# 10XGenomics/rust-pseudoaligner

Measured on AMD Instinct MI355X. Metric: reads/sec pseudoaligned (whole node) on synthetic 150bp reads, higher is better.
Workload: dtype u64; 1 GPU; config3: ~202k-transcript synthetic GENCODE-scale index (K=24), error-free 150bp reads; read_len=150, k=24, transcripts=201914, kmers=103866252, index_bytes=7185579820

## Files before the change

rust-pseudoaligner_amd/csrc/device_flatten.cpp:

```cpp
#include "device_flatten.hpp"

#include <algorithm>
#include <atomic>
#include <thread>

#include "dict_slots.hpp"
#include "lane_steps.hpp"
#include "pa_common.hpp"

#ifndef PA_BRANCH_TAILS
#define PA_BRANCH_TAILS 1
#endif

namespace pa {

DevIndexView FlatDevice::host_view() const {
    DevIndexView v;
    v.table = table.data();
    v.nbuckets = nbuckets;
    v.blobs = blobs.data();
    v.ledge = ledge.data();
    v.seg_g = seg_g.data();
    v.seg_nid = seg_nid.data();
    v.ec = ec.data();
    v.class_ref = class_ref.data();
    v.class_len = class_len.data();
    v.wtable = wtable.data();
    v.wbuckets = wbuckets;
    v.kmask = kmer_mask(k);
    v.kmask_hi = k > 32 ? kmer_mask(k - 32) : 0;
    v.k = k;
    v.num_nodes = num_nodes;
    v.num_classes = num_classes;
    v.num_segs = (uint32_t)seg_g.size();
    v.stream_nt = 0;
    v.bitmap_min = bitmap_min;
    v.bitmap_words = bitmap_words;
    return v;
}

namespace {

template <class F>
void par_ranges(int threads, uint64_t n, F f) {
    if (threads <= 1 || n < 4096) { f(0, n, 0); return; }
    std::vector<std::thread> th;
    for (int t = 0; t < threads; ++t) th.emplace_back([=] { f(n * t / threads, n * (t + 1) / threads, t); });
    for (auto& x : th) x.join();
}

template <class KT> struct Dict;

template <>
struct Dict<u128> {
    static constexpr double LOAD = 1.0 / 3.0;
    static constexpr uint32_t SLOTS = 2;
    uint32_t* words;
    uint64_t nbuckets;
    uint64_t bucket_of(u128 kmer) const { return ((pa_mix128((uint64_t)kmer, (uint64_t)(kmer >> 64)) >> 32) * (uint64_t)(uint32_t)nbuckets) >> 32; }
    void insert_mt(u128 kmer, uint32_t handle, uint32_t off) {
        uint64_t b = bucket_of(kmer);
        for (;;) {
            uint32_t* line = words + b * BUCKET_WORDS;
            for (uint32_t i = 0; i < SLOTS; ++i) {
                uint32_t expect = NO_HANDLE;
                if (__atomic_compare_exchange_n(&line[8 * i + 4], &expect, handle, false, __ATOMIC_RELAXED, __ATOMIC_RELAXED)) {
                    line[8 * i] = (uint32_t)kmer; line[8 * i + 1] = (uint32_t)(kmer >> 32);
                    line[8 * i + 2] = (uint32_t)(kmer >> 64); line[8 * i + 3] = (uint32_t)(kmer >> 96);
                    line[8 * i + 5] = off;
                    return;
                }
            }
            if (++b == nbuckets) b = 0;
        }
    }
    void insert_rest_mt(u128, uint32_t, uint32_t) {}
    bool find(u128 kmer, uint32_t& handle, uint32_t& off, uint32_t* probes_out = nullptr) const {
        uint64_t b = bucket_of(kmer);
        for (uint64_t probes = 0; probes < nbuckets; ++probes) {
            const uint32_t* line = words + b * BUCKET_WORDS;
            bool full = true;
            for (uint32_t i = 0; i < SLOTS; ++i) {
                if (line[8 * i + 4] == NO_HANDLE) { full = false; continue; }
                if (line[8 * i] == (uint32_t)kmer && line[8 * i + 1] == (uint32_t)(kmer >> 32) && line[8 * i + 2] == (uint32_t)(kmer >> 64) &&
                    line[8 * i + 3] == (uint32_t)(kmer >> 96)) {
                    handle = line[8 * i + 4];
                    off = line[8 * i + 5];
                    if (probes_out) *probes_out = (uint32_t)probes;
                    return true;
                }
            }
            if (!full) return false;
            if (++b == nbuckets) b = 0;
        }
        return false;
    }
};

struct HostAtomics {
    static bool cas(uint32_t* p, uint32_t expect, uint32_t v) { return __atomic_compare_exchange_n(p, &expect, v, false, __ATOMIC_RELAXED, __ATOMIC_RELAXED); }
    static void and_(uint32_t* p, uint32_t m) { __atomic_fetch_and(p, m, __ATOMIC_RELAXED); }
};

template <>
struct Dict<uint64_t> {
    static constexpr double LOAD = DICT_LOAD;
    static constexpr uint32_t SLOTS = SLOTS_PER_BUCKET;
    uint32_t* words;
    uint64_t nbuckets;
    void insert_mt(uint64_t kmer, uint32_t handle, uint32_t off) { dict_insert_home<HostAtomics>(words, (uint32_t)nbuckets, kmer, handle, off); }
    void insert_rest_mt(uint64_t kmer, uint32_t handle, uint32_t off) { dict_insert_rest<HostAtomics>(words, (uint32_t)nbuckets, kmer, handle, off); }
    bool find(uint64_t kmer, uint32_t& handle, uint32_t& off, uint32_t* probes_out = nullptr) const {
        uint32_t probes = 0;
        const bool found = dict_find64(words, (uint32_t)nbuckets, kmer, handle, off, probes);
        if (probes_out) *probes_out = probes;
        return found;
    }
};

}

template <class KT>
struct KmerMap {
    std::vector<KT> keys;
    std::vector<uint32_t> vals;
    uint64_t mask;
    explicit KmerMap(uint32_t n) {
        uint64_t cap = 16;
        while (cap < 2ull * n + 2) cap <<= 1;
        keys.assign(cap, 0);
        vals.assign(cap, NO_HANDLE);
        mask = cap - 1;
    }
    void insert(KT km, uint32_t v) {
        for (uint64_t j = KmerOps<KT>::hash(km) & mask;; j = (j + 1) & mask) {
            if (vals[j] == NO_HANDLE) { keys[j] = km; vals[j] = v; return; }
            if (keys[j] == km) return;
        }
    }
    uint32_t find(KT km) const {
        for (uint64_t j = KmerOps<KT>::hash(km) & mask;; j = (j + 1) & mask) {
            if (vals[j] == NO_HANDLE) return NO_HANDLE;
            if (keys[j] == km) return vals[j];
        }
    }
};

template <class KT>
static int flatten_t(const pa_flat_index& f, int threads, FlatDevice& out, bool device_dict) {
    if (threads < 1) threads = 1;
    const uint32_t k = f.k, N = f.num_nodes;
    out = FlatDevice();
    out.k = k;
    out.num_nodes = N;
    out.num_classes = f.num_classes;
    const KT mask = KmerOps<KT>::mask(k);
    const uint32_t topshift = 2 * (k - 1);

    if (f.num_transcripts >= 0xFFFFFFFFu) return fail(PA_ERR_UNSUPPORTED, "too many transcripts");
    std::vector<U4> cwin(f.num_classes, U4{0, 0, 0, 0});
    uint64_t nwin = 0;
    for (uint32_t c = 0; c < f.num_classes; ++c) {
        const uint32_t* ids = f.ec_ids + f.ec_offset[c];
        const uint64_t len = f.ec_offset[c + 1] - f.ec_offset[c];
        if (len == 0) continue;
        U4 w{ids[0], 0, 0, 0};
        uint64_t j = 0;
        for (; j < len && ids[j] - w.x < CLASS_WINDOW; ++j) w.y |= 1u << (ids[j] - w.x);
        if (j < len) {
            w.z = ids[j];
            for (; j < len && ids[j] - w.z < CLASS_WINDOW; ++j) w.w |= 1u << (ids[j] - w.z);
        }
        if (j < len) continue;
        cwin[c] = w;
        ++nwin;
    }
    uint32_t id_span = f.num_transcripts;
    for (uint64_t j = 0; j < f.ec_offset[f.num_classes]; ++j) id_span = std::max(id_span, f.ec_ids[j] + 1u);
    out.bitmap_words = ((id_span + 31) / 32 + 2 + 3) & ~3u;
    out.bitmap_min = 16;
    for (;;) {
        uint64_t n = 0;
        for (uint32_t c = 0; c < f.num_classes; ++c)
            n += cwin[c].y == 0 && f.ec_offset[c + 1] - f.ec_offset[c] >= out.bitmap_min;
        out.num_bitmaps = n;
        if (n * out.bitmap_words * 4ull <= (4ull << 30)) break;
        if (out.bitmap_min >= (1u << 24)) { out.bitmap_min = 0; out.num_bitmaps = 0; break; }
        out.bitmap_min *= 2;
    }
    out.class_ref.resize(f.num_classes);
    out.class_len.resize(f.num_classes);
    for (uint32_t c = 0; c < f.num_classes; ++c) {
        const uint64_t len = f.ec_offset[c + 1] - f.ec_offset[c];
        if (len >= 0xFFFFFFFFull || out.ec.size() / 4 >= 0xFFFFFFFFull) return fail(PA_ERR_UNSUPPORTED, "class id lists too large");
        out.class_ref[c] = (uint32_t)(out.ec.size() / 4);
        out.class_len[c] = (uint32_t)len;
        out.max_class_len = std::max(out.max_class_len, (uint32_t)len);
        out.ec.push_back(c);
        out.ec.insert(out.ec.end(), f.ec_ids + f.ec_offset[c], f.ec_ids + f.ec_offset[c + 1]);
        while (out.ec.size() % 4 || out.ec.size() - 4ull * out.class_ref[c] < 8) out.ec.push_back(0xFFFFFFFFu);
        if (out.bitmap_min && cwin[c].y == 0 && len >= out.bitmap_min) {
            const size_t at = out.ec.size();
            if (at != class_bitmap(out.class_ref[c], (uint32_t)len)) return fail(PA_ERR_INTERNAL, "class record of %llu ids is not %u chunks", (unsigned long long)len, class_record_chunks((uint32_t)len));
            out.ec.resize(at + out.bitmap_words, 0u);
            for (uint64_t j = f.ec_offset[c]; j < f.ec_offset[c + 1]; ++j) {
                out.ec[at + (f.ec_ids[j] >> 5)] |= 1u << (f.ec_ids[j] & 31u);
            }
        }
    }
    out.ec.resize(out.ec.size() + 8, 0xFFFFFFFFu);
    out.wbuckets = (uint32_t)std::max<uint64_t>(1, (uint64_t)((double)nwin / (WT_ENTRIES * 0.5)) + 1);
    out.wtable.assign((size_t)out.wbuckets * 16, 0);
    for (uint64_t l = 0; l < out.wbuckets; ++l) out.wtable[l * 16 + 4] = out.wtable[l * 16 + 9] = out.wtable[l * 16 + 14] = NO_CLASS;
    for (uint32_t c = 0; c < f.num_classes; ++c) {
        const U4 w = cwin[c];
        if (w.y == 0) continue;
        uint64_t line = ((uint64_t)window_hash(w.x, w.y, w.z, w.w) * out.wbuckets) >> 32;
        for (bool done = false; !done;) {
            uint32_t* e = out.wtable.data() + line * 16;
            for (uint32_t t = 0; t < WT_ENTRIES && !done; ++t)
                if (e[5 * t + 4] == NO_CLASS) {
                    e[5 * t] = w.x; e[5 * t + 1] = w.y; e[5 * t + 2] = w.z; e[5 * t + 3] = w.w; e[5 * t + 4] = c;
                    done = true;
                }
            if (++line == out.wbuckets) line = 0;
        }
    }

    std::vector<uint64_t> seq_pad(f.node_seq, f.node_seq + (f.seq_bases + 31) / 32);
    seq_pad.resize(seq_pad.size() + 3, 0);
    const uint64_t* node_seq = seq_pad.data();
    uint64_t nk = 0;
    for (uint32_t i = 0; i < N; ++i) {
        if (f.node_len[i] < k) return fail(PA_ERR_FORMAT, "node %u shorter than k", i);
        if (f.node_len[i] >= (1u << 24)) return fail(PA_ERR_UNSUPPORTED, "node %u longer than 2^24 bases", i);
        if (f.node_colour[i] >= f.num_classes) return fail(PA_ERR_FORMAT, "node %u: colour out of range", i);
        nk += f.node_len[i] - k + 1;
    }
    out.num_kmers = nk;
    std::vector<uint32_t> redge(4ull * N, NO_HANDLE), ledge_n(4ull * N, NO_HANDLE);
    {
        KmerMap<KT> first_of(N), last_of(N);
        if (!f.node_redge || !f.node_ledge)
            for (uint32_t i = 0; i < N; ++i) {
                first_of.insert(KmerOps<KT>::get(node_seq, f.node_start[i], k), i);
                last_of.insert(KmerOps<KT>::get(node_seq, f.node_start[i] + f.node_len[i] - k, k), i);
            }
        std::atomic<uint32_t> dangling{NO_HANDLE};
        par_ranges(threads, N, [&](uint64_t a, uint64_t b, int) {
            for (uint64_t i = a; i < b; ++i) {
                const uint64_t s = f.node_start[i];
                const KT first = KmerOps<KT>::get(node_seq, s, k), last = KmerOps<KT>::get(node_seq, s + f.node_len[i] - k, k);
                for (uint32_t base = 0; base < 4; ++base) {
                    if (f.node_exts[i] & (1u << base)) {
                        const uint32_t t = f.node_redge ? f.node_redge[4 * i + base] : first_of.find((last >> 2) | ((KT)base << topshift));
                        if (t >= N) dangling.store((uint32_t)i);
                        else redge[4 * i + base] = t;
                    }
                    if (f.node_exts[i] & (1u << (4 + base))) {
                        const uint32_t t = f.node_ledge ? f.node_ledge[4 * i + base] : last_of.find(((first << 2) | (KT)base) & mask);
                        if (t >= N) dangling.store((uint32_t)i);
                        else ledge_n[4 * i + base] = t;
                    }
                }
            }
        });
        if (dangling.load() != NO_HANDLE)
            return fail(PA_ERR_FORMAT, "node %u has an extension bit without a terminal neighbour k-mer (missing link)", dangling.load());
    }

    auto is_wide = [&](uint32_t i) { const U4 cw = cwin[f.node_colour[i]]; return cw.y == 0 || cw.w != 0; };
// ... 96 lines not shown
                const bool branch = (re & (re - 1)) != 0;
                uint32_t bn = NO_HANDLE;
                if (!branch) bn = redge[4 * cur + (uint32_t)__builtin_ctz(re)];
                else if (PA_BRANCH_TAILS) {
                    uint64_t best = 0;
                    for (uint32_t b = 0; b < 4; ++b) {
                        if (!(re & (1u << b))) continue;
                        const uint32_t t = redge[4 * cur + b];
                        const uint64_t c = 1 + shared_ids(f.node_colour[cur], f.node_colour[t]);
                        if (c > best) { best = c; bn = t; }
                    }
                }
                if (bn == NO_HANDLE) break;
                const uint64_t sb = (uint64_t)fin.back().e - (k - 1), full = sb + f.node_len[bn];
                if ((uint64_t)fin.back().e + 1 >= limit) break;
                const bool cut = full > limit;
                fin.back().branch = branch;
                if (!fits_after(fin, c0, SegI{bn, (uint32_t)sb, (uint32_t)(cut ? limit : full), cut})) { fin.back().branch = false; break; }
                if (cut) break;
                cur = bn;
            }
            for (const size_t c1 = c0 + (chain_first[c + 1] - chain_first[c]); fin.size() > c1 && !fin.back().link;) {
                const uint32_t re = f.node_exts[fin.back().node] & 15u;
                if (re == 0 || (re & (re - 1)) || out.node_s[redge[4 * fin.back().node + (uint32_t)__builtin_ctz(re)]] == 0) break;
                bool done = false;
                if (fin.back().e >= fin[fin.size() - 2].e + 2) {
                    SegI g = fin.back();
                    g.e -= 1;
                    g.link = true;
                    fin.pop_back();
                    done = fits_after(fin, c0, g);
                    if (!done) { g.e += 1; g.link = false; fin.push_back(g); }
                }
                if (!done) { fin.pop_back(); fin.back().branch = false; }
            }
        }
        fin_first.push_back((uint32_t)fin.size());
        segs.swap(fin);
        chain_first.swap(fin_first);
    }
    const size_t nsegs = segs.size();

    std::vector<uint32_t> chain_handle(nchains);
    out.seg_g.resize(nsegs);
    out.seg_nid.resize(nsegs);
    uint64_t cursor = 0;
    for (uint32_t c = 0; c < nchains; ++c) {
        if (cursor >= NO_HANDLE - 8) return fail(PA_ERR_UNSUPPORTED, "graph exceeds the 512 GiB chain address space");
        chain_handle[c] = (uint32_t)cursor;
        for (uint32_t t = chain_first[c]; t < chain_first[c + 1]; ++t) {
            out.seg_g[t] = ((uint64_t)cursor << CH_STRIDE_LOG2) + segs[t].s;
            out.seg_nid[t] = segs[t].node;
        }
        cursor += (segs[chain_first[c + 1] - 1].e + CH_STRIDE - 1) >> CH_STRIDE_LOG2;
    }
    for (uint32_t i = 0; i < N; ++i) out.handle[i] = chain_handle[out.handle[i]];
    const uint64_t nblocks = cursor;
    out.blobs.assign(nblocks * CH_BLOCK + 64, 0);

    std::atomic<uint32_t> bad_edge{NO_HANDLE}, bad_slots{NO_HANDLE};
    par_ranges(threads, nchains, [&](uint64_t ca, uint64_t cb, int) {
        std::vector<uint64_t> cs;
        for (uint64_t c = ca; c < cb; ++c) {
            const uint32_t t0 = chain_first[c], t1 = chain_first[c + 1], clen = segs[t1 - 1].e;
            cs.assign((clen + 31) / 32 + 9, 0);
            for (uint32_t t = t0; t < t1; ++t) {
                const SegI& g = segs[t];
                const uint64_t src = f.node_start[g.node];
                for (uint32_t o = t == t0 ? 0 : k - 1; g.s + o < g.e; ++o) set_base(cs.data(), g.s + o, get_base(node_seq, src + o));
            }
            const uint32_t nblk = (clen + CH_STRIDE - 1) >> CH_STRIDE_LOG2;
            uint32_t tlo = t0;
            for (uint32_t j = 0; j < nblk; ++j) {
                const uint32_t base = j << CH_STRIDE_LOG2;
                uint8_t* blk = out.blobs.data() + ((uint64_t)chain_handle[c] + j) * CH_BLOCK;
                uint32_t* sl = reinterpret_cast<uint32_t*>(blk);
                uint64_t* sq = reinterpret_cast<uint64_t*>(blk + CH_SEQ_BYTES);
                while (tlo < t1 && segs[tlo].e <= base) ++tlo;
                uint32_t slot = 0, recmask = 0;
                for (uint32_t t = tlo; t < t1 && segs[t].s < base + CH_WINDOW; ++t) {
                    const SegI& g = segs[t];
                    const U4 cw = cwin[f.node_colour[g.node]];
                    const bool wide = is_wide(g.node), last = t + 1 == t1, reach = g.e - base < CH_WINDOW,
                               edges = ((last && !g.link && has_redge(g.node)) || g.branch) && reach, link = last && g.link && reach;
                    if (slot + 1 + (wide ? 1 : 0) + (edges || link ? 1 : 0) > CH_SLOTS) { bad_slots.store(g.node); break; }
                    recmask |= 1u << slot;
                    uint32_t* r = sl + 4 * slot++;
                    r[0] = std::min<uint32_t>(g.e - base, SEG_E_FAR) | (wide ? SEG_WIDE : 0u) | (last ? SEG_LAST : 0u) | (edges ? SEG_EDGES : 0u) | (link ? SEG_LINK : 0u);
                    r[1] = f.node_colour[g.node]; r[2] = cw.x; r[3] = cw.y;
                    if (wide) {
                        uint32_t* x = sl + 4 * slot++;
                        x[0] = cw.z; x[1] = cw.w; x[2] = out.class_ref[f.node_colour[g.node]]; x[3] = out.class_len[f.node_colour[g.node]];
                    }
                    if (edges) {
                        uint32_t* x = sl + 4 * slot++;
                        for (uint32_t b = 0; b < 4; ++b) {
                            const uint32_t tn = redge[4 * g.node + b];
                            if (tn != NO_HANDLE && out.node_s[tn] != 0) bad_edge.store(g.node);
                            x[b] = tn == NO_HANDLE ? NO_HANDLE : out.handle[tn];
                        }
                    }
                    if (link) {
                        uint32_t* x = sl + 4 * slot++;
                        const uint32_t xt = out.node_s[g.node] + (g.e - g.s), adv = (xt - 1) >> CH_STRIDE_LOG2;
                        x[0] = out.handle[g.node] + adv;
                        x[1] = xt - (adv << CH_STRIDE_LOG2);
                        x[2] = x[3] = 0;
                    }
                }
                sl[0] |= (std::min(j, CH_BACK_MAX) << SEG_BACK_SHIFT) | (recmask << SEG_RECMASK_SHIFT);
                for (uint32_t w = 0; w < CH_WINDOW / 32; ++w) sq[w] = window32(cs.data(), base + 32ull * w);
            }
        }
    });
    if (bad_slots.load() != NO_HANDLE) return fail(PA_ERR_INTERNAL, "node %u: a chain block needs more than its four slots", bad_slots.load());
    par_ranges(threads, nblocks, [&](uint64_t ba, uint64_t bb, int) {
        for (uint64_t b = ba; b < bb; ++b) {
            uint32_t* sl = reinterpret_cast<uint32_t*>(out.blobs.data() + b * CH_BLOCK);
            const uint32_t recmask = sl[0] >> SEG_RECMASK_SHIFT;
            for (uint32_t t = 0; t < CH_SLOTS; ++t) {
                if (!((recmask >> t) & 1u) || !(sl[4 * t] & SEG_LINK)) continue;
                uint32_t* x = sl + 4 * (t + 1 + ((sl[4 * t] & SEG_WIDE) ? 1u : 0u));
                x[2] = of_cur(block_slot_of(out.blobs.data() + (uint64_t)x[0] * CH_BLOCK, x[1] - 1), true);
            }
        }
    });
    if (bad_edge.load() != NO_HANDLE) return fail(PA_ERR_FORMAT, "node %u: a right edge does not lead to the first k-mer of a chain", bad_edge.load());

    out.ledge.assign(8ull * nblocks + 8, NO_HANDLE);
    for (uint32_t c = 0; c < nchains; ++c) {
        const uint32_t a = segs[chain_first[c]].node;
        for (uint32_t b = 0; b < 4; ++b) {
            const uint32_t tn = ledge_n[4 * a + b];
            uint32_t* e = out.ledge.data() + 8ull * chain_handle[c] + 2 * b;
            e[1] = 0;
            if (tn == NO_HANDLE) continue;
            const uint32_t y = out.node_s[tn] + f.node_len[tn] - k;
            const uint32_t jy = y >> CH_STRIDE_LOG2, j = jy > CH_BACK_MAX ? jy - CH_BACK_MAX : 0;
            e[0] = out.handle[tn] + j;
            e[1] = y - (j << CH_STRIDE_LOG2) + 1;
        }
    }

    auto node_kmers = [&](uint32_t i, auto&& fn) {
        const uint64_t s = f.node_start[i];
        const uint32_t n = f.node_len[i] - k + 1;
        KT km = KmerOps<KT>::get(node_seq, s, k);
        for (uint32_t o = 0; o < n; ++o) {
            if (o) km = (km >> 2) | ((KT)get_base(node_seq, s + o + k - 1) << topshift);
            const uint32_t c = out.node_s[i] + o, blk = out.handle[i] + (c >> CH_STRIDE_LOG2);
            fn(km, blk, dict_entry_off(c, o == 0, block_slot_of(out.blobs.data() + (uint64_t)blk * CH_BLOCK, (c & (CH_STRIDE - 1)) + k - 1)));
        }
    };
    Dict<KT> dict{nullptr, 0};
    if (device_dict) {
        out.node_kcum.resize((size_t)N + 1);
        out.node_kcum[0] = 0;
        for (uint32_t i = 0; i < N; ++i) out.node_kcum[i + 1] = out.node_kcum[i] + (f.node_len[i] - k + 1);
    }
    double load0 = Dict<KT>::LOAD;
    if (const char* v = knob_str("PA_DICT_LOAD")) { const double x = atof(v); if (x > 0.01 && x <= 0.95) load0 = x; }
    for (double load = load0; !device_dict; load *= 0.75) {
        out.nbuckets = std::max<uint64_t>(1, (uint64_t)((double)nk / (Dict<KT>::SLOTS * load)) + 1);
        if (out.nbuckets >= 0xFFFFFFFFull) return fail(PA_ERR_UNSUPPORTED, "dictionary exceeds 2^32 buckets");
        out.table.assign(out.nbuckets * BUCKET_WORDS, 0xFFFFFFFFu);
        dict = Dict<KT>{out.table.data(), out.nbuckets};
        par_ranges(threads, N, [&](uint64_t a, uint64_t b, int) {
            for (uint64_t i = a; i < b; ++i) node_kmers((uint32_t)i, [&](KT km, uint32_t h, uint32_t o) { dict.insert_mt(km, h, o); });
        });
        par_ranges(threads, N, [&](uint64_t a, uint64_t b, int) {
            for (uint64_t i = a; i < b; ++i) node_kmers((uint32_t)i, [&](KT km, uint32_t h, uint32_t o) { dict.insert_rest_mt(km, h, o); });
        });
        std::atomic<uint32_t> bad{NO_HANDLE}, far{0};
        par_ranges(threads, N, [&](uint64_t a, uint64_t b, int) {
            for (uint64_t i = a; i < b; ++i)
                node_kmers((uint32_t)i, [&](KT km, uint32_t h, uint32_t o) {
                    uint32_t fh, fo, probes = 0;
                    if (!dict.find(km, fh, fo, &probes) || fh != h || fo != o) bad.store((uint32_t)i);
                    if (probes > DICT_MAX_PROBES) far.store(1);
                });
        });
        if (bad.load() != NO_HANDLE) return fail(PA_ERR_FORMAT, "a k-mer of node %u occurs twice in the graph", bad.load());
        if (!far.load()) break;
    }
    return PA_OK;
}

int flatten_for_device(const pa_flat_index& f, int threads, FlatDevice& out, bool device_dict) {
    if (f.k < PA_MIN_K || f.k > PA_MAX_K) return fail(PA_ERR_UNSUPPORTED, "k=%u outside [%u,%u]", f.k, PA_MIN_K, PA_MAX_K);
    return f.k <= 32 ? flatten_t<uint64_t>(f, threads, out, device_dict) : flatten_t<u128>(f, threads, out, device_dict);
}

}
```

rust-pseudoaligner_amd/csrc/device_flatten.hpp:

```cpp
#pragma once
#include <vector>

#include "device_layout.hpp"
#ifdef __HIPCC__
#include "hip_buffer.hpp"
#endif

namespace pa {

struct FlatDevice {
    std::vector<uint32_t> table;
    uint64_t nbuckets = 0;
    std::vector<uint8_t> blobs;
    std::vector<uint32_t> handle;
    std::vector<uint32_t> node_s;
    std::vector<uint32_t> ledge;
    std::vector<uint64_t> seg_g;
    std::vector<uint32_t> seg_nid;
    uint32_t num_chains = 0;
    std::vector<uint32_t> ec;
    std::vector<uint32_t> class_ref, class_len;
    std::vector<uint32_t> wtable;
    uint32_t wbuckets = 0;
    uint64_t num_kmers = 0;
    uint32_t k = 0, num_nodes = 0, num_classes = 0, max_class_len = 0;
    uint32_t bitmap_min = 0, bitmap_words = 0;
    uint64_t num_bitmaps = 0;
    std::vector<uint64_t> node_kcum;
    DevIndexView host_view() const;
};

int flatten_for_device(const pa_flat_index& f, int threads, FlatDevice& out, bool device_dict = false);

#ifdef __HIPCC__
int device_fill_index(const FlatDevice& fd, const uint8_t* d_blobs, DeviceBuffer<uint32_t>& table, uint64_t* nbuckets);
#endif

}
```

rust-pseudoaligner_amd/csrc/device_index.hip:

```cpp
#include <hip/hip_runtime.h>

#include <algorithm>
#include <cstdlib>
#include <cstring>
#include <map>
#include <memory>
#include <mutex>
#include <thread>

#include "device_flatten.hpp"
#include "hip_buffer.hpp"
#include "kernels.hpp"
#include "lane_steps.hpp"
#include "pa_common.hpp"
#include "synth_common.hpp"

using namespace pa;

namespace {

using Scratch = DeviceBuffer<uint8_t>;

int grow(Scratch& b, size_t need) { return b.reserve(need, need + need / 4 + 256); }

template <class T> int upload(DeviceBuffer<T>& dst, const T* src, size_t n) {
    const int e = dst.alloc(n ? n : 16 / sizeof(T));
    if (e != PA_OK) return e;
    if (n) PA_HIP_TRY(hipMemcpy(dst.get(), src, n * sizeof(T), hipMemcpyHostToDevice));
    return PA_OK;
}
template <class T> int upload(DeviceBuffer<T>& dst, const std::vector<T>& src) { return upload(dst, src.data(), src.size()); }

uint64_t list_hash_host(const uint32_t* v, uint32_t n) {
    uint64_t h = 0x243f6a8885a308d3ull ^ n;
    for (uint32_t i = 0; i < n; ++i) h = mix64(h ^ v[i]) + 0x9e3779b97f4a7c15ull;
    return h;
}

}

struct LaunchCtx {
    std::mutex mu;
    Scratch ctl;
    Scratch spill, trace, novel;
    Scratch keys, keys_sorted, keys_ctl;
    Scratch defer;
    uint32_t last_grid = 0;
    uint64_t last_arena_cap = 0;
    hipEvent_t ev0 = nullptr, ev1 = nullptr, ev2 = nullptr, ev3 = nullptr;
    bool timed = false;
    hipStream_t side = nullptr;
    hipEvent_t fork = nullptr, join = nullptr;
    void release() {
        if (side) (void)hipStreamSynchronize(side);
        for (Scratch* b : {&ctl, &spill, &trace, &novel, &keys, &keys_sorted, &keys_ctl, &defer}) b->release();
        for (hipEvent_t e : {ev0, ev1, ev2, ev3, fork, join})
            if (e) (void)hipEventDestroy(e);
        ev0 = ev1 = ev2 = ev3 = fork = join = nullptr;
        if (side) (void)hipStreamDestroy(side);
        side = nullptr;
        timed = false;
    }
};

struct pa_index {
    int device = 0;
    int num_cus = 0;
    DevIndexView dv{};
    DeviceBuffer<uint32_t> d_table, d_ledge, d_seg_nid, d_ec, d_class_ref, d_class_len, d_class_table, d_wtable;
    DeviceBuffer<uint8_t> d_blobs;
    DeviceBuffer<uint64_t> d_seg_g;
    uint64_t class_table_size = 0;
    pa_index_stats stats{};
    std::mutex mu;
    std::map<hipStream_t, std::shared_ptr<LaunchCtx>> ctxs;
    pa_overflow* ovf = nullptr;
    bool timing = false;
    std::mutex hmu;
    Scratch b_ascii, b_offsets, b_tiles, b_lens, b_results, b_arena, b_colour, b_nodes, b_nodes_len;
    std::vector<uint32_t> h_class_ids;
    std::vector<uint32_t> h_ec, h_class_ref, h_class_len;
    std::once_flag class_text_once;
    std::vector<uint64_t> h_class_text_off;
    std::vector<char> h_class_text;
    std::vector<uint32_t> h_arena;
    DeviceBuffer<uint64_t> d_class_text_off;
    DeviceBuffer<uint8_t> d_class_text;
    std::vector<std::pair<void*, void (*)(void*)>> ingest_caches;
    std::vector<std::pair<void*, void (*)(void*)>> host_pipes;
};

extern "C" {

int pa_device_count(void) {
    int n = 0;
    if (hipGetDeviceCount(&n) != hipSuccess) return 0;
    return n;
}

static int use_device(int device) {
    int n = 0;
    hipError_t e = hipGetDeviceCount(&n);
    if (e != hipSuccess || n <= 0)
        return fail(PA_ERR_NO_DEVICE, "no HIP device available (%s); this library has no CPU fallback",
                    e == hipSuccess ? "device count is 0" : hipGetErrorString(e));
    if (device < 0 || device >= n) return fail(PA_ERR_INVALID_ARG, "device %d out of range (have %d)", device, n);
    PA_HIP_TRY(hipSetDevice(device));
    return PA_OK;
}

extern "C++" {
namespace pa {
void index_host_classes(const pa_index* idx, const uint32_t** ec, const uint32_t** class_ref, int* device) {
    *ec = idx->h_ec.data();
    *class_ref = idx->h_class_ref.data();
    *device = idx->device;
}
void index_host_class_text(pa_index* idx, const uint64_t** off, const char** text) {
    std::call_once(idx->class_text_once, [idx] {
        const uint32_t nc = idx->stats.num_classes;
        const uint32_t* ec = idx->h_ec.data();
        const uint32_t* cref = idx->h_class_ref.data();
        auto digits = [](uint32_t v) { uint32_t d = 1; while (v >= 10) { v /= 10; ++d; } return d; };
        std::vector<uint64_t>& off_v = idx->h_class_text_off;
        off_v.assign((size_t)nc + 1, 0);
        const int T = std::max(1, std::min(16, usable_threads()));
        const uint32_t* clen = idx->h_class_len.data();
        auto ids_of = [&](uint32_t c, const uint32_t*& ids, uint32_t& n) {
            ids = ec + 4ull * cref[c] + 1;
            n = clen[c];
        };
        {
            std::vector<std::thread> th;
            for (int t = 0; t < T; ++t)
                th.emplace_back([&, t] {
                    for (uint64_t c = (uint64_t)nc * t / T; c < (uint64_t)nc * (t + 1) / T; ++c) {
                        const uint32_t* ids; uint32_t n;
                        ids_of((uint32_t)c, ids, n);
                        uint64_t len = n ? 2ull * (n - 1) : 0;
                        for (uint32_t j = 0; j < n; ++j) len += digits(ids[j]);
                        off_v[c + 1] = len;
                    }
                });
            for (auto& x : th) x.join();
        }
        for (uint32_t c = 0; c < nc; ++c) off_v[c + 1] += off_v[c];
        idx->h_class_text.resize(off_v[nc] + 16);
        {
            std::vector<std::thread> th;
            for (int t = 0; t < T; ++t)
                th.emplace_back([&, t] {
                    for (uint64_t c = (uint64_t)nc * t / T; c < (uint64_t)nc * (t + 1) / T; ++c) {
                        const uint32_t* ids; uint32_t n;
                        ids_of((uint32_t)c, ids, n);
                        char* o = idx->h_class_text.data() + off_v[c];
                        for (uint32_t j = 0; j < n; ++j) {
                            if (j) { *o++ = ','; *o++ = ' '; }
                            char b[10]; int k = 10; uint32_t v = ids[j];
                            do { b[--k] = (char)('0' + v % 10); v /= 10; } while (v);
                            memcpy(o, b + k, (size_t)(10 - k)); o += 10 - k;
                        }
                    }
                });
            for (auto& x : th) x.join();
        }
    });
    *off = idx->h_class_text_off.data();
    *text = idx->h_class_text.data();
}
int index_device_class_text(pa_index* idx, const uint64_t** d_off, const uint8_t** d_text) {
    const uint64_t* off = nullptr;
    const char* txt = nullptr;
    index_host_class_text(idx, &off, &txt);
    std::lock_guard<std::mutex> g(idx->mu);
    if (!idx->d_class_text.get()) {
        if (hipSetDevice(idx->device) != hipSuccess) return fail(PA_ERR_HIP, "hipSetDevice failed");
        int e = upload(idx->d_class_text_off, off, idx->h_class_text_off.size());
        if (e == PA_OK) e = upload(idx->d_class_text, reinterpret_cast<const uint8_t*>(txt), idx->h_class_text.size());
        if (e != PA_OK) return e;
    }
    *d_off = idx->d_class_text_off.get();
    *d_text = idx->d_class_text.get();
    return PA_OK;
}
void* index_take_ingest_cache(pa_index* idx) {
    std::lock_guard<std::mutex> g(idx->mu);
    if (idx->ingest_caches.empty()) return nullptr;
    void* c = idx->ingest_caches.back().first;
    idx->ingest_caches.pop_back();
    return c;
}
void* index_take_host_pipe(pa_index* idx) {
    std::lock_guard<std::mutex> g(idx->mu);
    if (idx->host_pipes.empty()) return nullptr;
    void* c = idx->host_pipes.back().first;
    idx->host_pipes.pop_back();
    return c;
}
void index_put_host_pipe(pa_index* idx, void* pipe, void (*free_fn)(void*)) {
    {
        std::lock_guard<std::mutex> g(idx->mu);
        if (idx->host_pipes.size() < 2) {
            idx->host_pipes.emplace_back(pipe, free_fn);
            return;
        }
    }
    free_fn(pipe);
}
void index_put_ingest_cache(pa_index* idx, void* cache, void (*free_fn)(void*)) {
    {
        std::lock_guard<std::mutex> g(idx->mu);
        if (idx->ingest_caches.size() < 4) {
            idx->ingest_caches.emplace_back(cache, free_fn);
            return;
        }
    }
    free_fn(cache);
}
}
}

void pa_index_destroy(pa_index* idx) {
    if (!idx) return;
    (void)hipSetDevice(idx->device);
    {
        std::vector<std::pair<void*, void (*)(void*)>> parked;
        { std::lock_guard<std::mutex> g(idx->mu); parked.swap(idx->ingest_caches); parked.insert(parked.end(), idx->host_pipes.begin(), idx->host_pipes.end()); idx->host_pipes.clear(); }
        for (auto& c : parked) c.second(c.first);
    }
    for (auto& kv : idx->ctxs) kv.second->release();
    delete idx;
}

int pa_index_create(const pa_flat_index* flat, int device, pa_index** out) {
    if (!flat || !out) return fail(PA_ERR_INVALID_ARG, "null argument");
    int rc = use_device(device);
    if (rc != PA_OK) return rc;
    FlatDevice fd;
    int threads = usable_threads();
    if (threads < 1) threads = 1;
    rc = flatten_for_device(*flat, threads, fd, true);
    if (rc != PA_OK) return rc;

    std::vector<uint32_t> ctab((size_t)fd.num_classes * 2 + 16, 0xFFFFFFFFu);
    for (uint32_t c = 0; c < fd.num_classes; ++c) {
        uint64_t j = list_hash_host(fd.ec.data() + 4ull * fd.class_ref[c] + 1, fd.class_len[c]) % ctab.size();
        while (ctab[j] != 0xFFFFFFFFu)
            if (++j == ctab.size()) j = 0;
        ctab[j] = c;
    }

    pa_index* idx = new (std::nothrow) pa_index();
    if (!idx) return fail(PA_ERR_OOM, "out of memory");
    idx->device = device;
    hipDeviceProp_t prop;
    if (hipGetDeviceProperties(&prop, device) == hipSuccess) idx->num_cus = prop.multiProcessorCount;
    if (idx->num_cus <= 0) idx->num_cus = 256;
    rc = upload(idx->d_blobs, fd.blobs);
    if (rc == PA_OK) rc = upload(idx->d_ledge, fd.ledge);
    if (rc == PA_OK) rc = device_fill_index(fd, idx->d_blobs.get(), idx->d_table, &fd.nbuckets);
    if (rc == PA_OK) rc = upload(idx->d_seg_g, fd.seg_g);
    if (rc == PA_OK) rc = upload(idx->d_seg_nid, fd.seg_nid);
    if (rc == PA_OK) rc = upload(idx->d_ec, fd.ec);
    if (rc == PA_OK) rc = upload(idx->d_class_ref, fd.class_ref);
    if (rc == PA_OK) rc = upload(idx->d_class_len, fd.class_len);
    if (rc == PA_OK) rc = upload(idx->d_class_table, ctab);
    if (rc == PA_OK) rc = upload(idx->d_wtable, fd.wtable);
    if (rc != PA_OK) { pa_index_destroy(idx); return rc; }
    idx->class_table_size = ctab.size();
    idx->dv = fd.host_view();
    idx->dv.table = idx->d_table.get();
    idx->dv.blobs = idx->d_blobs.get();
    idx->dv.ledge = idx->d_ledge.get();
    idx->dv.seg_g = idx->d_seg_g.get();
    idx->dv.seg_nid = idx->d_seg_nid.get();
    idx->h_ec = fd.ec;
    idx->h_class_ref = fd.class_ref;
    idx->h_class_len = fd.class_len;
    idx->dv.ec = idx->d_ec.get();
    idx->dv.class_ref = idx->d_class_ref.get();
    idx->dv.class_len = idx->d_class_len.get();
    idx->dv.wtable = idx->d_wtable.get();
    idx->dv.stream_nt = (fd.k <= 32 && fd.nbuckets * BUCKET_WORDS * 4 > (512ull << 20)) ? 1u : 0u;
    pa_index_stats& s = idx->stats;
    s.num_kmers = fd.num_kmers;
    s.table_slots = fd.nbuckets * SLOTS_PER_BUCKET;
    s.bytes_table = fd.nbuckets * BUCKET_WORDS * 4;
    s.bytes_graph = fd.blobs.size() + fd.ledge.size() * 4 + fd.seg_g.size() * 12;
    s.bytes_classes = (fd.ec.size() + fd.class_ref.size() + fd.class_len.size() + ctab.size() + fd.wtable.size()) * 4;
    s.bytes_total = s.bytes_table + s.bytes_graph + s.bytes_classes;
    s.num_nodes = fd.num_nodes;
    s.num_classes = fd.num_classes;
    s.k = fd.k;
    s.max_class_len = fd.max_class_len;
    *out = idx;
    return PA_OK;
}

int pa_index_create_multi(const pa_flat_index* flat, const int* devices, int ndev, pa_index** out) {
    if (!flat || !devices || !out || ndev < 1) return fail(PA_ERR_INVALID_ARG, "null argument or ndev < 1");
    for (int i = 0; i < ndev; ++i) out[i] = nullptr;
    for (int i = 0; i < ndev; ++i) {
        for (int j = 0; j < i; ++j)
            if (devices[j] == devices[i]) {
                for (int t = 0; t < i; ++t) { pa_index_destroy(out[t]); out[t] = nullptr; }
                return fail(PA_ERR_INVALID_ARG, "device %d listed twice", devices[i]);
            }
        const int rc = pa_index_create(flat, devices[i], &out[i]);
        if (rc != PA_OK) {
            const std::string why = last_error_ref();
            for (int t = 0; t <= i; ++t) { pa_index_destroy(out[t]); out[t] = nullptr; }
            return fail(rc, "device %d: %s", devices[i], why.c_str());
        }
    }
    return PA_OK;
}

int pa_index_get_stats(const pa_index* idx, pa_index_stats* stats) {
    if (!idx || !stats) return fail(PA_ERR_INVALID_ARG, "null argument");
    *stats = idx->stats;
    return PA_OK;
}

uint32_t pa_words_per_read(uint32_t max_read_len) { return (max_read_len + 31) / 32 ? (max_read_len + 31) / 32 : 1; }
size_t pa_tiles_words(uint64_t n_reads, uint32_t words_per_read) { return (size_t)((n_reads + 63) / 64) * words_per_read * 64; }

int pa_encode_reads_device(const pa_index* idx, const uint8_t* d_ascii, const uint64_t* d_offsets, uint64_t n_reads,
                           uint32_t words_per_read, uint64_t* d_tiles, uint32_t* d_lens, void* stream) {
    if (!idx || !d_ascii || !d_offsets || !d_tiles || !d_lens || words_per_read == 0) return fail(PA_ERR_INVALID_ARG, "null argument");
    PA_HIP_TRY(hipSetDevice(idx->device));
    const int e = launch_encode(d_ascii, d_offsets, n_reads, words_per_read, d_tiles, d_lens, static_cast<hipStream_t>(stream));
    if (e) return fail(PA_ERR_HIP, "encode launch: %s", hipGetErrorString((hipError_t)e));
    return PA_OK;
}

static int env_int(const char* name, int dflt) { return knob_int(name, dflt); }

static uint32_t spill_cap_of(uint32_t wpr) { return 256 * wpr + 24; }

static int pool_geometry(pa_index* idx, uint64_t n_reads, uint32_t wpr, uint32_t* grid, size_t* lds, uint32_t* slots) {
    const size_t cu_lds = 160 * 1024 - 4096;
    int per_cu = env_int("PA_MAP_BLOCKS_PER_CU", 3);
    uint32_t S = 0;
    for (; per_cu >= 1; --per_cu) {
        const size_t per_wave = cu_lds / (size_t)per_cu / (PA_MAP_BLOCK / 64);
        const size_t per_slot = pool_slot_bytes(wpr);
        if (per_wave < pool_fixed_bytes() + 64 * per_slot + 16) continue;
        S = (uint32_t)((per_wave - pool_fixed_bytes() - 16) / per_slot);
        break;
    }
    if (S < 64) return fail(PA_ERR_UNSUPPORTED, "reads of %u words do not fit the LDS of a compute unit", wpr);
    if (S > pool_max_slots()) S = pool_max_slots();
    const int want = env_int("PA_POOL_SLOTS", 0);
    if (want >= 64 && (uint32_t)want <= S) S = (uint32_t)want;
    *slots = S;
    *lds = pool_lds_bytes(wpr, S);
    int occ = 0;
    if (pool_kernel_occupancy(*lds, &occ) == 0 && occ >= 1 && occ < per_cu) per_cu = occ;
    const uint64_t ntiles = (n_reads + 63) / 64;
    const uint64_t waves_wanted = (ntiles + 7) / 8;
    uint64_t blocks = (waves_wanted + PA_MAP_BLOCK / 64 - 1) / (PA_MAP_BLOCK / 64);
    const uint64_t cap = (uint64_t)idx->num_cus * per_cu;
    if (blocks > cap) blocks = cap;
    if (blocks < 1) blocks = 1;
    *grid = (uint32_t)blocks;
    return PA_OK;
}

static int ctx_of(pa_index* idx, hipStream_t stream, std::shared_ptr<LaunchCtx>* out) {
    std::lock_guard<std::mutex> g(idx->mu);
    auto it = idx->ctxs.find(stream);
    if (it == idx->ctxs.end()) {
        std::shared_ptr<LaunchCtx> c(new (std::nothrow) LaunchCtx());
        if (!c) return fail(PA_ERR_OOM, "out of memory");
        const int rc = grow(c->ctl, 1024);
        if (rc != PA_OK) return rc;
        it = idx->ctxs.emplace(stream, std::move(c)).first;
    }
    *out = it->second;
    return PA_OK;
}

static int map_launch_locked(pa_index* idx, LaunchCtx* cx, const uint64_t* d_tiles, const uint32_t* d_lens, uint64_t n_reads, uint32_t wpr,
                             uint32_t allowed, pa_read_result* d_results, uint32_t* d_arena, uint64_t arena_cap, uint32_t* d_colour,
                             uint64_t* d_counts, uint32_t* d_nodes, uint32_t* d_nodes_len, hipStream_t stream, uint32_t uniform_len = 0) {
    if (n_reads >= 0xFFFFFFFFull) return fail(PA_ERR_UNSUPPORTED, "at most 2^32-2 reads per batch");
    if (wpr == 0 || wpr > (PA_MAX_READ_LEN + 31) / 32) return fail(PA_ERR_UNSUPPORTED, "words_per_read %u outside [1,%u]", wpr, (PA_MAX_READ_LEN + 31) / 32);
    uint32_t grid = 0;
    size_t lds = 0;
    uint32_t slots = 64;
    int rc = pool_geometry(idx, n_reads, wpr, &grid, &lds, &slots);
    if (rc != PA_OK) return rc;
    const uint32_t spill_cap = spill_cap_of(wpr);
    {
        const size_t per_block = (size_t)(PA_MAP_BLOCK / 64) * slots * spill_cap * 4 * (d_nodes ? 2 : 1);
        const size_t budget = (size_t)6 << 30;
        if ((size_t)grid * per_block > budget) grid = (uint32_t)std::max<size_t>(1, budget / per_block);
    }
    const size_t lanes = (size_t)grid * (PA_MAP_BLOCK / 64) * slots;
    rc = grow(cx->spill, lanes * spill_cap * 4);
    if (rc != PA_OK) return rc;
    if (d_nodes) { rc = grow(cx->trace, lanes * spill_cap * 4); if (rc != PA_OK) return rc; }
    PA_HIP_TRY(hipMemsetAsync(cx->ctl.get(), 0, 512, stream));
    MapParams p{};
    p.ix = idx->dv;
    p.tiles = d_tiles;
    p.lens = d_lens;
    p.uniform_len = uniform_len;
    p.n_reads = n_reads;
    p.wpr = wpr;
    p.allowed = allowed;
    p.results = d_results;
    p.arena = d_arena;
    p.arena_cap = arena_cap > PA_MAX_ARENA_ENTRIES ? PA_MAX_ARENA_ENTRIES : arena_cap;
    p.colour_out = d_colour;
    p.arena_top = cx->ctl.as<unsigned long long>();
    p.status = cx->ctl.as<uint32_t>() + 2;
    p.tile_ctr = cx->ctl.as<uint32_t>() + 3;
    p.spill = cx->spill.as<uint32_t>();
    p.spill_cap = spill_cap;
    const uint64_t counts_len = (uint64_t)idx->stats.num_classes + 3;
    const uint64_t defer_cap = defer_capacity(n_reads, grid * (PA_MAP_BLOCK / 64));
    if ((rc = grow(cx->defer, defer_cap * 32))) return rc;
    p.defer = cx->defer.as<uint32_t>();
    p.defer_top = cx->ctl.as<unsigned long long>() + 58;
    p.defer_cap = defer_cap;
    p.keys_cap = 0;
    uint64_t keys_cap = 0;
    if (d_counts) {
        keys_cap = key_stream_capacity(n_reads, grid * (PA_MAP_BLOCK / 64));
        size_t sorted_bytes = 0, ctl_bytes = 0;
        count_keys_scratch(counts_len, n_reads, keys_cap, defer_cap, &sorted_bytes, &ctl_bytes);
        if ((rc = grow(cx->keys, (keys_cap + defer_cap) * 4)) || (rc = grow(cx->keys_sorted, sorted_bytes)) || (rc = grow(cx->keys_ctl, ctl_bytes))) return rc;
        p.keys = cx->keys.as<uint32_t>();
        p.keys_top = cx->ctl.as<unsigned long long>() + 57;
        p.keys_cap = keys_cap;
        p.counts = reinterpret_cast<unsigned long long*>(d_counts);
    }
    p.class_table = idx->d_class_table.get();
    p.class_table_size = idx->class_table_size;
    p.pool_slots = slots;
    p.dbg = env_int("PA_MAP_STATS", 0) ? cx->ctl.as<unsigned long long>() + 2 : nullptr;
    p.ablate = (uint32_t)env_int("PA_MAP_ABLATE", 0);
    pa_overflow* ovf = nullptr;
    { std::lock_guard<std::mutex> g(idx->mu); ovf = idx->ovf; }
    if (d_counts && ovf) {
        const uint64_t want = n_reads + 64;
        rc = grow(cx->novel, want * 8);
// ... 517 lines not shown
```

rust-pseudoaligner_amd/csrc/device_layout.hpp:

```cpp
#pragma once
#include <cstdint>

#include "../../include/pseudoaligner_amd.h"

#if defined(__HIPCC__)
#include <hip/hip_runtime.h>
#define PA_HD __host__ __device__ __forceinline__
#else
#define PA_HD inline
#endif

namespace pa {

constexpr uint32_t NO_HANDLE = 0xFFFFFFFFu;
constexpr uint32_t CH_BLOCK = 128;
constexpr uint32_t CH_STRIDE_LOG2 = 6;
constexpr uint32_t CH_STRIDE = 1u << CH_STRIDE_LOG2;
constexpr uint32_t CH_WINDOW = 256;
constexpr uint32_t CH_SLOTS = 4;
constexpr uint32_t CH_SEQ_BYTES = 64;
constexpr uint32_t CH_BACK_MAX = 3;
constexpr uint32_t SEG_E_MASK = 0xFFFFu, SEG_E_FAR = 0xFFFFu;
constexpr uint32_t SEG_WIDE = 1u << 16, SEG_LAST = 1u << 17, SEG_EDGES = 1u << 18, SEG_LINK = 1u << 19;
constexpr uint32_t CH_TAIL = 128;
constexpr uint32_t SEG_BACK_SHIFT = 20, SEG_RECMASK_SHIFT = 28;
constexpr uint32_t ENT_P_MASK = 63u, ENT_NODE_START = 64u, ENT_BACK_SHIFT = 7, ENT_CUR_SHIFT = 9;
PA_HD uint32_t block_slot_of(const uint8_t* blk, uint32_t y) {
    const uint32_t* sl = reinterpret_cast<const uint32_t*>(blk);
    const uint32_t recmask = sl[0] >> SEG_RECMASK_SHIFT;
    for (uint32_t t = 0; t < CH_SLOTS; ++t)
        if (((recmask >> t) & 1u) && (sl[4 * t] & SEG_E_MASK) > y) return t;
    return 0;
}
PA_HD uint32_t dict_entry_off(uint32_t c, bool node_start, uint32_t slot) {
    const uint32_t j = c >> CH_STRIDE_LOG2;
    return (c & ENT_P_MASK) | (node_start ? ENT_NODE_START : 0u) | ((j < CH_BACK_MAX ? j : CH_BACK_MAX) << ENT_BACK_SHIFT) | (slot << ENT_CUR_SHIFT);
}
constexpr uint32_t CLASS_WINDOW = 32;
constexpr uint32_t SLOTS_PER_BUCKET = 4;
constexpr uint32_t BUCKET_WORDS = 16;
constexpr uint32_t SLOT_WORDS = 4;
constexpr uint32_t SLOT_OFF_MASK = 0xFFFFFFu;
constexpr uint32_t SLOT_FLAG_SHIFT = 24;
constexpr uint32_t SLOT_FLAG_OVERFLOW = 8u;
constexpr double DICT_LOAD = 0.25;
constexpr uint32_t DICT_MAX_PROBES = 15;

struct alignas(16) U4 {
    uint32_t x, y, z, w;
};
struct alignas(8) Q2 {
    uint64_t a, b;
};

constexpr uint32_t WT_ENTRIES = 3;

struct DevIndexView {
    const uint32_t* table;
    uint64_t nbuckets;
    const uint8_t* blobs;
    const uint32_t* ledge;
    const uint64_t* seg_g;
    const uint32_t* seg_nid;
    const uint32_t* ec;
    const uint32_t* class_ref;
    const uint32_t* class_len;
    const uint32_t* wtable;
    uint32_t wbuckets;
    uint64_t kmask;
    uint64_t kmask_hi;
    uint32_t k;
    uint32_t num_nodes, num_classes;
    uint32_t num_segs;
    uint32_t stream_nt;
    uint32_t bitmap_min;
    uint32_t bitmap_words;
};

PA_HD uint32_t class_record_chunks(uint32_t len) { return len < 4 ? 2u : (len + 4) >> 2; }
PA_HD uint64_t class_bitmap(uint32_t ref, uint32_t len) { return 4ull * ((uint64_t)ref + class_record_chunks(len)); }

}
```

rust-pseudoaligner_amd/csrc/dict_slots.hpp:

```cpp
#pragma once
#include "lane_steps.hpp"

namespace pa {

template <class A>
PA_HD bool slot_claim(uint32_t* slot, uint64_t km, uint32_t handle, uint32_t off) {
    if (!A::cas(slot + 2, NO_HANDLE, handle)) return false;
    slot[0] = (uint32_t)km;
    slot[1] = (uint32_t)(km >> 32);
    A::and_(slot + 3, off | ~SLOT_OFF_MASK);
    return true;
}

template <class A>
PA_HD void dict_insert_home(uint32_t* table, uint32_t nbuckets, uint64_t km, uint32_t handle, uint32_t off) {
    uint32_t home;
    const uint32_t b = pa_bucket_home(km, nbuckets, home);
    slot_claim<A>(table + (uint64_t)b * BUCKET_WORDS + SLOT_WORDS * home, km, handle, off);
}

template <class A>
PA_HD void dict_insert_rest(uint32_t* table, uint32_t nbuckets, uint64_t km, uint32_t handle, uint32_t off) {
    uint32_t home;
    uint32_t b = pa_bucket_home(km, nbuckets, home);
    {
        const uint32_t* hs = table + (uint64_t)b * BUCKET_WORDS + SLOT_WORDS * home;
        if (hs[2] != NO_HANDLE && hs[0] == (uint32_t)km && hs[1] == (uint32_t)(km >> 32)) return;
    }
    for (bool first = true;; first = false) {
        uint32_t* line = table + (uint64_t)b * BUCKET_WORDS;
        uint32_t* hs = line + SLOT_WORDS * home;
        if (!first && slot_claim<A>(hs, km, handle, off)) return;
        for (uint32_t i = 0; i < 3; ++i)
            if (slot_claim<A>(line + SLOT_WORDS * ((home + 1 + i) & 3u), km, handle, off)) {
                A::and_(hs + 3, ~(1u << (SLOT_FLAG_SHIFT + i)));
                return;
            }
        A::and_(hs + 3, ~(SLOT_FLAG_OVERFLOW << SLOT_FLAG_SHIFT));
        if (++b == nbuckets) b = 0;
    }
}

PA_HD bool dict_find64(const uint32_t* table, uint32_t nbuckets, uint64_t km, uint32_t& handle, uint32_t& off, uint32_t& probes) {
    uint32_t home;
    uint32_t b = pa_bucket_home(km, nbuckets, home);
    const uint32_t klo = (uint32_t)km, khi = (uint32_t)(km >> 32);
    for (probes = 0; probes < nbuckets; ++probes) {
        const uint32_t* line = table + (uint64_t)b * BUCKET_WORDS;
        const U4 v = *reinterpret_cast<const U4*>(line + SLOT_WORDS * home);
        if (slot_holds(v, klo, khi)) { handle = v.z; off = v.w & SLOT_OFF_MASK; return true; }
        const uint32_t fl = slot_flags(v);
        for (uint32_t c = fl & 7u; c; c &= c - 1) {
            const U4 v2 = *reinterpret_cast<const U4*>(line + SLOT_WORDS * ((home + 1 + pa_ctz32(c)) & 3u));
            if (slot_holds(v2, klo, khi)) { handle = v2.z; off = v2.w & SLOT_OFF_MASK; return true; }
        }
        if (!(fl & SLOT_FLAG_OVERFLOW)) return false;
        if (++b == nbuckets) b = 0;
    }
    return false;
}

}
```

rust-pseudoaligner_amd/csrc/index_fill.hip:

```cpp
#include <hip/hip_runtime.h>
#include <cstdlib>

#include <algorithm>

#include "device_flatten.hpp"
#include "dict_slots.hpp"
#include "hip_buffer.hpp"
#include "lane_steps.hpp"
#include "pa_common.hpp"

namespace pa {
namespace {

__device__ __forceinline__ uint64_t win32(const uint64_t* w, uint32_t pos) {
    const uint32_t i = pos >> 5, s = (pos & 31) * 2;
    return s ? (w[i] >> s) | (w[i + 1] << (64 - s)) : w[i];
}

template <class KT> struct FillOps;
template <> struct FillOps<uint64_t> {
    static constexpr uint32_t SLOTS = SLOTS_PER_BUCKET;
    static constexpr double LOAD = DICT_LOAD;
    __host__ __device__ static uint64_t mask(uint32_t k) { return k >= 32 ? ~0ull : ((1ull << (2 * k)) - 1); }
    __device__ static uint64_t get(const uint64_t* seq, uint32_t o, uint32_t k) { return win32(seq, o) & mask(k); }
};
struct DeviceAtomics {
    __device__ static bool cas(uint32_t* p, uint32_t expect, uint32_t v) { return atomicCAS(p, expect, v) == expect; }
    __device__ static void and_(uint32_t* p, uint32_t m) { atomicAnd(p, m); }
};
template <> struct FillOps<u128> {
    static constexpr uint32_t SLOTS = 2;
    static constexpr double LOAD = 1.0 / 3.0;
    __host__ __device__ static u128 mask(uint32_t k) { return k >= 64 ? ~(u128)0 : (((u128)1 << (2 * k)) - 1); }
    __device__ static u128 get(const uint64_t* seq, uint32_t o, uint32_t k) {
        return ((u128)(win32(seq, o + 32) & FillOps<uint64_t>::mask(k - 32)) << 64) | win32(seq, o);
    }
    __device__ static uint32_t bucket(u128 km, uint32_t nbuckets) { return __umulhi((uint32_t)(pa_mix128((uint64_t)km, (uint64_t)(km >> 64)) >> 32), nbuckets); }
    __device__ static bool try_insert(uint32_t* line, u128 km, uint32_t handle, uint32_t off) {
        for (uint32_t i = 0; i < 2; ++i)
            if (atomicCAS(line + 8 * i + 4, NO_HANDLE, handle) == NO_HANDLE) {
                line[8 * i] = (uint32_t)km; line[8 * i + 1] = (uint32_t)(km >> 32);
                line[8 * i + 2] = (uint32_t)(km >> 64); line[8 * i + 3] = (uint32_t)(km >> 96);
                line[8 * i + 5] = off;
                return true;
            }
        return false;
    }
    __device__ static int look(const uint32_t* line, u128 km, uint32_t& handle, uint32_t& off) {
        bool full = true;
        for (uint32_t i = 0; i < 2; ++i) {
            if (line[8 * i + 4] == NO_HANDLE) { full = false; continue; }
            if (line[8 * i] == (uint32_t)km && line[8 * i + 1] == (uint32_t)(km >> 32) && line[8 * i + 2] == (uint32_t)(km >> 64) &&
                line[8 * i + 3] == (uint32_t)(km >> 96)) {
                handle = line[8 * i + 4];
                off = line[8 * i + 5];
                return 1;
            }
        }
        return full ? 2 : 0;
    }
};

template <class KT>
__device__ __forceinline__ bool dict_find(const uint32_t* table, uint32_t nbuckets, KT km, uint32_t& handle, uint32_t& off, uint32_t& probes);
template <>
__device__ __forceinline__ bool dict_find<uint64_t>(const uint32_t* table, uint32_t nbuckets, uint64_t km, uint32_t& handle, uint32_t& off, uint32_t& probes) {
    return dict_find64(table, nbuckets, km, handle, off, probes);
}
template <>
__device__ __forceinline__ bool dict_find<u128>(const uint32_t* table, uint32_t nbuckets, u128 km, uint32_t& handle, uint32_t& off, uint32_t& probes) {
    uint32_t b = FillOps<u128>::bucket(km, nbuckets);
    for (probes = 0; probes < nbuckets; ++probes) {
        const int r = FillOps<u128>::look(table + (uint64_t)b * BUCKET_WORDS, km, handle, off);
        if (r != 2) return r == 1;
        if (++b == nbuckets) b = 0;
    }
    return false;
}

struct KmerAt {
    uint32_t node, block, off;
    const uint64_t* seq;
    uint32_t rel;
};

__device__ __forceinline__ uint32_t node_of_kmer(const uint64_t* kcum, uint32_t num_nodes, uint64_t g) {
    uint32_t lo = 0, hi = num_nodes - 1;
    while (lo < hi) {
        const uint32_t mid = lo + (hi - lo + 1) / 2;
        if (kcum[mid] <= g) lo = mid; else hi = mid - 1;
    }
    return lo;
}

__device__ __forceinline__ KmerAt kmer_at(const uint8_t* blobs, const uint32_t* handle, const uint32_t* node_s, const uint64_t* kcum, uint32_t num_nodes, uint64_t g, uint32_t k) {
    KmerAt a;
    a.node = node_of_kmer(kcum, num_nodes, g);
    const uint32_t o = (uint32_t)(g - kcum[a.node]), c = node_s[a.node] + o;
    a.block = handle[a.node] + (c >> CH_STRIDE_LOG2);
    a.off = dict_entry_off(c, o == 0, block_slot_of(blobs + (uint64_t)a.block * CH_BLOCK, (c & (CH_STRIDE - 1)) + k - 1));
    a.seq = reinterpret_cast<const uint64_t*>(blobs + (uint64_t)a.block * CH_BLOCK + CH_SEQ_BYTES);
    a.rel = c & (CH_STRIDE - 1);
    return a;
}

template <class KT>
__global__ __launch_bounds__(256) void pa_fill_insert_kernel(const uint8_t* __restrict__ blobs, const uint32_t* __restrict__ handle, const uint32_t* __restrict__ node_s,
                                                             const uint64_t* __restrict__ kcum, uint32_t num_nodes, uint64_t nk, uint32_t k, uint32_t* table,
                                                             uint32_t nbuckets, int pass) {
    const uint64_t g = (uint64_t)blockIdx.x * blockDim.x + threadIdx.x;
    if (g >= nk) return;
    const KmerAt a = kmer_at(blobs, handle, node_s, kcum, num_nodes, g, k);
    const KT km = FillOps<KT>::get(a.seq, a.rel, k);
    if constexpr (sizeof(KT) == 8) {
        if (pass == 0) dict_insert_home<DeviceAtomics>(table, nbuckets, km, a.block, a.off);
        else dict_insert_rest<DeviceAtomics>(table, nbuckets, km, a.block, a.off);
    } else {
        if (pass != 0) return;
        uint32_t b = FillOps<KT>::bucket(km, nbuckets);
        for (;;) {
            if (FillOps<KT>::try_insert(table + (uint64_t)b * BUCKET_WORDS, km, a.block, a.off)) return;
            if (++b == nbuckets) b = 0;
        }
    }
}

template <class KT>
__global__ __launch_bounds__(256) void pa_fill_verify_kernel(const uint8_t* __restrict__ blobs, const uint32_t* __restrict__ handle, const uint32_t* __restrict__ node_s,
                                                             const uint64_t* __restrict__ kcum, uint32_t num_nodes, uint64_t nk, uint32_t k,
                                                             const uint32_t* __restrict__ table, uint32_t nbuckets, uint32_t* __restrict__ flags) {
    const uint64_t g = (uint64_t)blockIdx.x * blockDim.x + threadIdx.x;
    if (g >= nk) return;
    const KmerAt a = kmer_at(blobs, handle, node_s, kcum, num_nodes, g, k);
    const KT km = FillOps<KT>::get(a.seq, a.rel, k);
    uint32_t fh = 0, fo = 0, probes = 0;
    if (!dict_find<KT>(table, nbuckets, km, fh, fo, probes) || fh != a.block || fo != a.off) atomicMin(flags, a.node);
    if (probes > DICT_MAX_PROBES) flags[1] = 1;
}

template <class KT>
int fill_t(const FlatDevice& fd, const uint8_t* d_blobs, DeviceBuffer<uint32_t>& table_out, uint64_t* nbuckets_out) {
    const uint32_t N = fd.num_nodes, k = fd.k;
    const uint64_t nk = fd.num_kmers;
    DeviceBuffer<uint32_t> table, d_handle, d_node_s, d_flags;
    DeviceBuffer<uint64_t> d_kcum;
    int e = d_handle.alloc(N ? N : 1);
    if (e == PA_OK) e = d_node_s.alloc(N ? N : 1);
    if (e == PA_OK) e = d_kcum.alloc((size_t)N + 1);
    if (e == PA_OK) e = d_flags.alloc(4);
    if (e != PA_OK) return e;
    if (N) PA_HIP_TRY(hipMemcpy(d_handle.get(), fd.handle.data(), (size_t)N * 4, hipMemcpyHostToDevice));
    if (N) PA_HIP_TRY(hipMemcpy(d_node_s.get(), fd.node_s.data(), (size_t)N * 4, hipMemcpyHostToDevice));
    PA_HIP_TRY(hipMemcpy(d_kcum.get(), fd.node_kcum.data(), ((size_t)N + 1) * 8, hipMemcpyHostToDevice));
    uint64_t nbuckets = 0;
    double load0 = FillOps<KT>::LOAD;
    {
        size_t free_b = 0, total_b = 0;
        const double dense = sizeof(KT) == 8 ? 0.5 : FillOps<KT>::LOAD;
        if (load0 < dense && hipMemGetInfo(&free_b, &total_b) == hipSuccess && (double)nk / (FillOps<KT>::SLOTS * load0) * BUCKET_WORDS * 4 > (double)free_b / 4) load0 = dense;
    }
    if (const char* v = knob_str("PA_DICT_LOAD")) { const double x = atof(v); if (x > 0.01 && x <= 0.95) load0 = x; }
    for (double load = load0;; load *= 0.75) {
        nbuckets = std::max<uint64_t>(1, (uint64_t)((double)nk / (FillOps<KT>::SLOTS * load)) + 1);
        if (nbuckets >= 0xFFFFFFFFull) return fail(PA_ERR_UNSUPPORTED, "dictionary exceeds 2^32 buckets");
        if ((e = table.alloc(nbuckets * BUCKET_WORDS)) != PA_OK) return e;
        PA_HIP_TRY(hipMemsetAsync(table.get(), 0xFF, nbuckets * BUCKET_WORDS * 4, nullptr));
        const uint32_t init[4] = {NO_HANDLE, 0u, NO_HANDLE, NO_HANDLE};
        PA_HIP_TRY(hipMemcpy(d_flags.get(), init, 16, hipMemcpyHostToDevice));
        if (nk) {
            const dim3 grid((uint32_t)((nk + 255) / 256));
            for (int pass = 0; pass < (sizeof(KT) == 8 ? 2 : 1); ++pass) {
                hipLaunchKernelGGL(pa_fill_insert_kernel<KT>, grid, dim3(256), 0, nullptr, d_blobs, d_handle.get(), d_node_s.get(), d_kcum.get(), N, nk, k,
                                   table.get(), (uint32_t)nbuckets, pass);
                PA_HIP_TRY(hipGetLastError());
            }
            hipLaunchKernelGGL(pa_fill_verify_kernel<KT>, grid, dim3(256), 0, nullptr, d_blobs, d_handle.get(), d_node_s.get(), d_kcum.get(), N, nk, k,
                               table.get(), (uint32_t)nbuckets, d_flags.get());
            PA_HIP_TRY(hipGetLastError());
        }
        uint32_t flags[4];
        PA_HIP_TRY(hipMemcpy(flags, d_flags.get(), 16, hipMemcpyDeviceToHost));
        if (flags[0] != NO_HANDLE) return fail(PA_ERR_FORMAT, "a k-mer of node %u occurs twice in the graph", flags[0]);
        if (!flags[1]) break;
    }
    *nbuckets_out = nbuckets;
    table_out = std::move(table);
    return PA_OK;
}

}

int device_fill_index(const FlatDevice& fd, const uint8_t* d_blobs, DeviceBuffer<uint32_t>& table, uint64_t* nbuckets) {
    return fd.k <= 32 ? fill_t<uint64_t>(fd, d_blobs, table, nbuckets) : fill_t<u128>(fd, d_blobs, table, nbuckets);
}

}
```

rust-pseudoaligner_amd/csrc/lane_steps_body.hpp:

```cpp
#if PA_LS_COMMON
enum : uint32_t { ST_EMPTY = 0, ST_SEEK = 1, ST_FWD = 2, ST_LEFT = 3, ST_ISECT = 4, ST_NONE = 5,
                  ST_F_LIGHT = 6, ST_F_SCAN = 7, ST_F_COOP = 8, ST_F_BITS = 9, ST_F_MASK = 10, ST_COUNT = 11 };
enum : uint32_t { F_FRESH = 1u, F_FIRST_SEEK = 2u, F_LEFT_SEED = 4u, F_SPILL_OVERFLOW = 8u, F_CAREFUL = 16u, F_LISTS = 32u,
                  F_SMALL_BASE = 64u,
                  F_SPEC = 128u };
constexpr uint32_t NO_CLASS = 0xFFFFFFFFu;
constexpr uint32_t LDS_CLASSES = 4;
#endif

#if PA_LS_LANE
#if !PA_LANE_WIDE
struct Lane {
    uint32_t rid;
    uint32_t lk;
    uint32_t cm;
    uint32_t h;
    uint32_t of;
    uint32_t rr;
    uint32_t rm;
    uint32_t ph;
    uint32_t nc;
};
constexpr uint32_t LANE_MAX_READ_LEN = 16383u;
PA_HD uint32_t l_L(const Lane& s) { return s.lk & 0x3FFFu; }
// ... 288 lines not shown

PA_HD uint32_t window_class(const DevIndexView& ix, uint32_t b1, uint32_t m1, uint32_t b2, uint32_t m2) {
#if defined(__HIP_DEVICE_COMPILE__)
    uint32_t line = __umulhi(window_hash(b1, m1, b2, m2), ix.wbuckets);
#else
    uint32_t line = (uint32_t)(((uint64_t)window_hash(b1, m1, b2, m2) * ix.wbuckets) >> 32);
#endif
    for (;;) {
        const U4* p = reinterpret_cast<const U4*>(ix.wtable + (uint64_t)line * 16);
        const U4 a = p[0], b = p[1], c = p[2], d = p[3];
        if (a.x == b1 && a.y == m1 && a.z == b2 && a.w == m2 && b.x != NO_CLASS) return b.x;
        if (b.y == b1 && b.z == m1 && b.w == b2 && c.x == m2 && c.y != NO_CLASS) return c.y;
        if (c.z == b1 && c.w == m1 && d.x == b2 && d.y == m2 && d.z != NO_CLASS) return d.z;
        if (b.x == NO_CLASS || c.y == NO_CLASS || d.z == NO_CLASS) return NO_CLASS;
        if (++line == ix.wbuckets) line = 0;
    }
}

PA_HD uint32_t window_bits(const uint32_t* bits, uint32_t b) {
    const uint32_t w = b >> 5, sh = b & 31u;
    const uint64_t v = (uint64_t)bits[w] | ((uint64_t)bits[w + 1] << 32);
    return (uint32_t)(v >> sh);
}

PA_HD uint32_t window_at(uint32_t b, uint32_t c, uint32_t n) {
    const uint32_t d = CLASS_WINDOW + b - c;
    const uint32_t r = (uint32_t)(((uint64_t)n << 32) >> (d & 63u));
    return d - 1u < 63u ? r : 0u;
}
#endif

#if PA_LS_LANE
template <bool TRACE>
PA_HD bool push_node(Lane& s, ColRef c, const DevIndexView& ix, const Seg& hd, uint64_t gpos) {
    if (TRACE) {
        const uint32_t nt = l_ntrace(s);
        if (nt < c.spill_cap) c.trace[nt] = trace_nid(ix, gpos);
        l_inc_trace(s);
    }
    const uint32_t n = l_ncol(s);
    if (!(l_flags(s) & F_LISTS)) {
        if (hd.cmask == 0) {
            const uint32_t np = n >> 1;
            if (np >= PEND_MAX || 2 * np + 1 >= c.spill_cap) return true;
            c.pend[2 * np] = hd.ec_ref;
            c.pend[2 * np + 1] = hd.ec_len;
            s.nc += 2;
            return false;
        }
        U4 w = *reinterpret_cast<const U4*>(c.win);
        uint32_t cand = hd.cid;
        if (!(n & 1u)) {
            w = U4{hd.cmin, hd.cmask, hd.cmin2, hd.cmask2};
        } else {
            const uint32_t m1 = w.y & (window_at(w.x, hd.cmin, hd.cmask) | window_at(w.x, hd.cmin2, hd.cmask2));
            const uint32_t m2 = w.w & (window_at(w.z, hd.cmin, hd.cmask) | window_at(w.z, hd.cmin2, hd.cmask2));
            if (pa_popc32(m1) + pa_popc32(m2) != pa_popc32(hd.cmask) + pa_popc32(hd.cmask2))
                cand = (m1 == w.y && m2 == w.w) ? c.wcand[0] : NO_CLASS;
            w.y = m1;
            w.w = m2;
        }
        *reinterpret_cast<U4*>(c.win) = w;
        c.wcand[0] = cand;
        s.nc |= 1u;
        return false;
    }
    const bool wide = (hd.flags & SEG_WIDE) != 0;
    const uint32_t ec_ref = wide ? hd.ec_ref : ix.class_ref[hd.cid], ec_len = wide ? hd.ec_len : pa_popc32(hd.cmask);
    U4 r = *reinterpret_cast<const U4*>(c.win);
    const bool dup = (n > 0 && r.x == ec_ref) | (n > 1 && r.y == ec_ref) | (n > 2 && r.z == ec_ref) | (n > 0 && r.w == ec_ref);
    if (dup) return false;
    if (n == 0) r.x = ec_ref;
    if (n == 1) r.y = ec_ref;
    if (n == 2) r.z = ec_ref;
    if (n == 0 || ec_len < c.wcand[0]) {
        r.w = ec_ref;
        c.wcand[0] = ec_len;
        if (ec_len <= 8) l_or_flags(s, F_SMALL_BASE);
    }
    *reinterpret_cast<U4*>(c.win) = r;
    if (n < LDS_CLASSES) {
        c.refs[n] = ec_ref;
        c.lens[n] = ec_len;
        c.cids[n] = hd.cid;
    } else {
        const uint32_t o = 4 * (n - LDS_CLASSES);
        if (o + 3 >= c.spill_cap || n >= NC_COL_MASK) { l_or_flags(s, F_SPILL_OVERFLOW); return false; }
        c.spill[o] = ec_ref;
        c.spill[o + 1] = ec_len;
        c.spill[o + 2] = hd.cid;
    }
    s.nc += 1;
    return false;
}

PA_HD void lane_start(Lane& s, uint32_t rid, uint32_t L, uint32_t k) {
    s.rid = rid;
    l_zero(s);
    l_set_lk(s, L, 0, L < k ? ST_NONE : ST_SEEK);
    s.of = F_FIRST_SEEK << 24;
}
PA_HD void restart_lists(Lane& s, uint32_t k) {
    lane_start(s, s.rid, l_L(s), k);
    l_or_flags(s, F_LISTS);
}
PA_HD uint32_t window_todo(const Lane& s) {
    const uint32_t n = l_ncol(s);
    return (n >> 1) == 0 ? 0u : (n & 1u) ? 1u : 2u;
}
#endif
#if PA_LS_COMMON
PA_HD void list_window_mask(const DevIndexView& ix, uint32_t ref, uint32_t len, uint32_t b1, uint32_t b2, uint32_t& m1, uint32_t& m2) {
    const uint32_t* ids = ix.ec + 4ull * ref + 1;
    m1 = m2 = 0;
    for (uint32_t j = 0; j < len; ++j) {
        const uint32_t d1 = ids[j] - b1, d2 = ids[j] - b2;
        if (d1 < CLASS_WINDOW) m1 |= 1u << d1;
        if (d2 < CLASS_WINDOW) m2 |= 1u << d2;
    }
#if !defined(__HIP_DEVICE_COMPILE__)
    if (ix.bitmap_min && len >= ix.bitmap_min) {
        const uint32_t* bits = ix.ec + class_bitmap(ref, len);
        const uint32_t x1 = window_bits(bits, b1), x2 = window_bits(bits, b2);
        if (x1 != m1 || x2 != m2) { m1 = m2 = 0xDEADBEEFu; }
    }
#endif
}
#endif
#if PA_LS_LANE
PA_HD void mask_pending(Lane& s, const DevIndexView& ix, ColRef c) {
    U4 w = *reinterpret_cast<const U4*>(c.win);
    const uint32_t np = l_npend(s);
    uint32_t a1 = w.y, a2 = w.w;
    for (uint32_t i = 0; i < np; ++i) {
        uint32_t m1, m2;
        list_window_mask(ix, c.pend[2 * i], c.pend[2 * i + 1], w.x, w.z, m1, m2);
        a1 &= m1;
        a2 &= m2;
    }
    if (a1 != w.y || a2 != w.w) c.wcand[0] = NO_CLASS;
    w.y = a1;
    w.w = a2;
    *reinterpret_cast<U4*>(c.win) = w;
    s.nc = (s.nc & ~NC_COL_MASK) | 1u;
}
#endif

#if PA_LS_COMMON
struct SeekProbe {
    U4 v;
    uint32_t klo, khi;
    uint32_t pending;
};
struct SeekProbe2 {
    U4 k0, v0, k1, v1;
    uint32_t w0, w1, w2, w3;
};
constexpr uint32_t SK_NAMED = 7u, SK_FULL = 8u, SK_MASK = 15u;
PA_HD uint32_t pa_bucket_home(uint64_t kmer, uint32_t nbuckets, uint32_t& home) {
    uint32_t x = (uint32_t)kmer * 0x9E3779B1u + (uint32_t)(kmer >> 32) * 0x85EBCA77u;
    x ^= x >> 15;
    x *= 0x2C1B3C6Du;
    x ^= x >> 13;
    home = x & 3u;
#if defined(__HIP_DEVICE_COMPILE__)
    return __umulhi(x, nbuckets);
#else
    return (uint32_t)(((uint64_t)x * nbuckets) >> 32);
#endif
}
#endif
#if PA_LS_LANE
PA_HD bool seek_two(const Lane& s, uint32_t K) { return (l_flags(s) & F_SPEC) && l_probe(s) == 0 && l_kp(s) + PA_SEEK_STRIDE <= l_L(s) - K; }
PA_HD uint32_t l_pending(const Lane& s) { return s.rm & SK_MASK; }
PA_HD void seek_issue(const Lane& s, const DevIndexView& ix, ReadRef rd, SeekProbe& q, uint32_t ahead = 0, bool live = true) {
    const uint32_t at = live ? l_kp(s) + ahead : l_kp(s);
    const uint64_t kmer = read_window_in(rd, at) & ix.kmask;
    uint32_t home;
    uint32_t b = pa_bucket_home(kmer, (uint32_t)ix.nbuckets, home) + (ahead ? 0u : l_probe(s));
    if (b >= (uint32_t)ix.nbuckets) b -= (uint32_t)ix.nbuckets;
    q.pending = ahead ? 0u : l_pending(s);
    const uint32_t named = q.pending & SK_NAMED;
    uint32_t slot = named ? (home + 1u + pa_ctz32(named)) & 3u : home;
    if (!live) { b = 0; slot = 0; }
    q.v = ld_stream(reinterpret_cast<const U4*>(ix.table + (uint64_t)b * BUCKET_WORDS + SLOT_WORDS * slot), (PA_NT & 4) || ix.stream_nt);
    q.klo = (uint32_t)kmer;
    q.khi = (uint32_t)(kmer >> 32);
}
#endif
#if PA_LS_COMMON
PA_HD bool slot_holds(const U4& v, uint32_t klo, uint32_t khi) { return v.z != NO_HANDLE && v.x == klo && v.y == khi; }
PA_HD uint32_t slot_flags(const U4& v) { return (~v.w >> SLOT_FLAG_SHIFT) & 15u; }
#endif
#if PA_LS_LANE
PA_HD void seek_finish(Lane& s, uint32_t K, uint32_t h, uint32_t off, bool full, uint32_t probe);
#endif
#if PA_LS_COMMON
PA_HD void seek_eval(const SeekProbe& q, uint32_t& h, uint32_t& off, bool& full, uint32_t& pending) {
    h = NO_HANDLE;
    off = 0;
    const bool hit = slot_holds(q.v, q.klo, q.khi);
    if (hit) { h = q.v.z; off = q.v.w & SLOT_OFF_MASK; }
    const uint32_t named = q.pending & SK_NAMED;
    const uint32_t next = named ? (named & (named - 1u)) | (q.pending & SK_FULL) : slot_flags(q.v);
    pending = hit ? 0u : (next & SK_NAMED) ? next : 0u;
    full = (next & SK_FULL) != 0;
}
#endif
#if PA_LS_LANE
PA_HD bool seek_settle(Lane& s, uint32_t K, const SeekProbe& q, bool more) {
    uint32_t h, off, pending;
    bool full;
    seek_eval(q, h, off, full, pending);
    if (pending) { s.rm = (s.rm & ~SK_MASK) | pending; return true; }
    const uint32_t probe = l_probe(s);
    if (!more || h != NO_HANDLE || (full && probe < DICT_MAX_PROBES)) {
        seek_finish(s, K, h, off, full, probe);
        return true;
    }
    l_set_kp(s, l_kp(s) + PA_SEEK_STRIDE);
    s.rm &= ~SK_MASK;
    s.nc &= ~(15u << NC_PROBE_SHIFT);
    return false;
}
PA_HD void seek_complete(Lane& s, uint32_t K, const SeekProbe& q) { (void)seek_settle(s, K, q, false); }
PA_HD void seek_complete2(Lane& s, uint32_t K, const SeekProbe& q0, bool two, const SeekProbe& q1) {
    if (seek_settle(s, K, q0, two)) return;
    (void)seek_settle(s, K, q1, false);
}
PA_HD void seek_finish(Lane& s, uint32_t K, uint32_t h, uint32_t off, bool full, uint32_t probe) {
    const uint32_t L = l_L(s), kp = l_kp(s);
    s.nc &= ~(15u << NC_PROBE_SHIFT);
    s.rm &= ~SK_MASK;
    if (h != NO_HANDLE) {
        s.h = h;
        const uint32_t fl = l_flags(s), p = (off & ENT_P_MASK) | of_cur((off >> ENT_CUR_SHIFT) & 3u, true);
        const uint32_t thr = L / 5;
        if ((fl & F_FIRST_SEEK) && kp >= thr) {
            const uint32_t back = (off >> ENT_BACK_SHIFT) & CH_BACK_MAX;
            l_set_left_ra(s, kp);
            s.ph = h - back;
            s.rr = (off & ENT_P_MASK) + CH_STRIDE * back + ((off & ENT_NODE_START) ? 1u : 0u);
            s.of = p | (((fl & ~(F_FIRST_SEEK | F_SPEC)) | F_FRESH | F_LEFT_SEED) << 24);
            l_set_st(s, ST_LEFT);
        } else {
            s.of = p | (((fl & ~(F_FIRST_SEEK | F_SPEC)) | F_FRESH) << 24);
            l_set_st(s, ST_FWD);
        }
        return;
    }
    if (full && probe < DICT_MAX_PROBES) {
        s.nc |= (probe + 1) << NC_PROBE_SHIFT;
        return;
    }
    const uint32_t nkp = kp + PA_SEEK_STRIDE;
    l_set_kp(s, nkp);
    l_or_flags(s, F_SPEC);
    if (nkp > L - K) l_set_st(s, l_ncol(s) ? ST_ISECT : ST_NONE);
}
#endif

#if PA_LS_COMMON
PA_HD uint64_t pa_mix128(uint64_t lo, uint64_t hi) { return pa_mix64(lo ^ (pa_mix64(hi) * 0x9e3779b97f4a7c15ull)); }
#endif

#if PA_LS_LANE
PA_HD void seek_issue_k2(const Lane& s, const DevIndexView& ix, ReadRef rd, SeekProbe2& q) {
    const uint32_t kp = l_kp(s), probe = l_probe(s);
    const uint64_t klo = read_window(rd, kp), khi = read_window(rd, kp + 32) & ix.kmask_hi;
#if defined(__HIP_DEVICE_COMPILE__)
    uint32_t b = __umulhi((uint32_t)(pa_mix128(klo, khi) >> 32), (uint32_t)ix.nbuckets) + probe;
#else
    uint32_t b = (uint32_t)(((pa_mix128(klo, khi) >> 32) * (uint32_t)ix.nbuckets) >> 32) + probe;
#endif
    if (b >= (uint32_t)ix.nbuckets) b -= (uint32_t)ix.nbuckets;
    const U4* line = reinterpret_cast<const U4*>(ix.table + (uint64_t)b * BUCKET_WORDS);
    q.k0 = line[0]; q.v0 = line[1]; q.k1 = line[2]; q.v1 = line[3];
    q.w0 = (uint32_t)klo; q.w1 = (uint32_t)(klo >> 32); q.w2 = (uint32_t)khi; q.w3 = (uint32_t)(khi >> 32);
}
PA_HD void seek_complete_k2(Lane& s, uint32_t K, const SeekProbe2& q) {
    const bool h0 = q.k0.x == q.w0 && q.k0.y == q.w1 && q.k0.z == q.w2 && q.k0.w == q.w3 && q.v0.x != NO_HANDLE,
               h1 = q.k1.x == q.w0 && q.k1.y == q.w1 && q.k1.z == q.w2 && q.k1.w == q.w3 && q.v1.x != NO_HANDLE;
    seek_finish(s, K, h0 ? q.v0.x : h1 ? q.v1.x : NO_HANDLE, h0 ? q.v0.y : q.v1.y, q.v0.x != NO_HANDLE && q.v1.x != NO_HANDLE, l_probe(s));
}
PA_HD void seek_step(Lane& s, const DevIndexView& ix, ReadRef rd) {
    const uint32_t K = ix.k;
    if (K > 32) {
        SeekProbe2 q2;
        seek_issue_k2(s, ix, rd, q2);
        seek_complete_k2(s, K, q2);
        return;
    }
    SeekProbe q, q1;
    const bool two = seek_two(s, K);
    seek_issue(s, ix, rd, q);
    seek_issue(s, ix, rd, q1, PA_SEEK_STRIDE, two);
    seek_complete2(s, K, q, two, q1);
}
#endif

#if PA_LS_COMMON
struct FwdLoad {
    U4 s0, s1, s2, s3;
    Q2 s01, s23, s45;
};
#endif
#if PA_LS_LANE
PA_HD void fwd_issue(const Lane& s, const DevIndexView& ix, FwdLoad& f) {
    const uint32_t K = ix.k, L = l_L(s);
    const bool fresh = l_flags(s) & F_FRESH;
    const uint32_t xs = l_off(s) + (fresh ? K : 0u);
    const uint32_t kp0 = l_kp(s) + (fresh ? K : 0u);
    const uint8_t* blk = chain_block(ix, s.h);
    const U4* sp = reinterpret_cast<const U4*>(blk);
    const uint32_t rot = l_cur(s);
    f.s0 = PA_LD(8, sp + rot); f.s1 = PA_LD(8, sp + ((rot + 1) & 3u)); f.s2 = PA_LD(8, sp + ((rot + 2) & 3u)); f.s3 = PA_LD(8, sp + ((rot + 3) & 3u));
    const uint32_t most = pa_min(L - kp0, 128u), nwords = ((xs & 31) + most + 31) >> 5;
    const Q2* sq2 = reinterpret_cast<const Q2*>(blk + CH_SEQ_BYTES + 8u * (xs >> 5));
    f.s01 = PA_LD(8, sq2);
    f.s23 = f.s45 = Q2{0ull, 0ull};
    if (nwords > 2) f.s23 = PA_LD(8, sq2 + 1);
    if (nwords > 4) f.s45 = PA_LD(8, sq2 + 2);
}
#endif

#if PA_LS_COMMON
struct DiffMasks {
    uint64_t m0, m1, m2, m3;
    uint32_t p0, p1, p2, p3;
};
PA_HD uint64_t diff_word(const DiffMasks& d, uint32_t w) { return sel4q(w, d.m0, d.m1, d.m2, d.m3); }
PA_HD uint32_t mism_prefix(const DiffMasks& d, uint32_t z) {
    const uint32_t w = z >> 5, r = z & 31u;
    const uint32_t b03 = sel4(w, 0u, d.p0, d.p1, d.p2), base = (w & 4u) ? d.p3 : b03;
    return base + pa_popc64(diff_word(d, w) & ((1ull << (2 * r)) - 1));
}
#endif

#if PA_LS_LANE
template <bool TRACE = false>
PA_HD void fwd_finish_general(Lane& s, const DevIndexView& ix, ReadRef rd, ColRef cols, uint32_t allowed, const FwdLoad& f) {
    const uint32_t K = ix.k, L = l_L(s);
    const uint32_t fl = l_flags(s);
    const bool fresh = fl & F_FRESH, careful = fl & F_CAREFUL;
    uint32_t x = l_off(s) + (fresh ? K : 0u);
    uint32_t kp = l_kp(s) + (fresh ? K : 0u);
    const uint32_t xs = x, kp0 = kp;
    uint32_t snp = s.rr >> 24, cov = l_cov(s), mism = l_mism(s);
    const uint32_t most = pa_min(L - kp0, 128u), nwords = ((xs & 31) + most + 31) >> 5;
    const uint64_t a[5] = {f.s01.a, f.s01.b, nwords > 2 ? f.s23.a : 0ull, nwords > 2 ? f.s23.b : 0ull, nwords > 4 ? f.s45.a : 0ull};
    const Slots sl{f.s0, f.s1, f.s2, f.s3};
    const bool known = s.of & OF_CUR_KNOWN;
    const uint32_t rot = l_cur(s);
    uint32_t cur = known ? 0u : seg_find(sl, x - 1);
    Seg g = seg_at(sl, cur);
    if (fresh) {
        cov += K;
        if (push_node<TRACE>(s, cols, ix, g, 64ull * s.h + l_off(s))) {
            restart_lists(s, K);
            return;
        }
        snp = 0;
    }
    uint64_t r[5];
    {
        const uint32_t i0 = (kp0 >> 5) * rd.stride, ilast = (rd.wmax - 1) * rd.stride;
#pragma unroll
        for (uint32_t i = 0; i < 5; ++i) r[i] = rd.p[pa_min(i0 + i * rd.stride, ilast)];
    }
    const uint32_t sh_a = (xs & 31) * 2, sh_r = (kp0 & 31) * 2;
    DiffMasks dm;
    dm.m0 = diff_mask(funnel(r[0], r[1], sh_r) ^ funnel(a[0], a[1], sh_a), 32u);
    dm.m1 = most > 32u ? diff_mask(funnel(r[1], r[2], sh_r) ^ funnel(a[1], a[2], sh_a), 32u) : 0ull;
    dm.m2 = most > 64u ? diff_mask(funnel(r[2], r[3], sh_r) ^ funnel(a[2], a[3], sh_a), 32u) : 0ull;
    dm.m3 = most > 96u ? diff_mask(funnel(r[3], r[4], sh_r) ^ funnel(a[3], a[4], sh_a), 32u) : 0ull;
    dm.p0 = pa_popc64(dm.m0); dm.p1 = dm.p0 + pa_popc64(dm.m1); dm.p2 = dm.p1 + pa_popc64(dm.m2); dm.p3 = dm.p2 + pa_popc64(dm.m3);
    const uint32_t lim = careful ? 32u : 128u;
    uint32_t consumed = 0, st = ST_FWD, h = s.h, nfl = fl & ~F_FRESH;
    uint32_t ncur = 0xFFFFFFFFu;
    bool premature = false, hopped = false;
    for (;;) {
        const uint32_t n = pa_min(pa_min(g.e - x, L - kp), lim - consumed);
        uint32_t matched;
        if (!careful) {
            const uint32_t cnt = mism_prefix(dm, consumed + n) - mism_prefix(dm, consumed);
            if (snp + cnt > allowed) { nfl |= F_CAREFUL; break; }
            snp += cnt;
            mism += cnt;
            matched = n;
        } else {
            matched = compare_chunk(n ? dm.m0 & (~0ull >> (64u - 2u * n)) : 0ull, n, allowed, snp, mism, premature);
        }
        x += matched; kp += matched; cov += matched; consumed += matched;
        if (premature) { nfl &= ~F_CAREFUL; st = kp > L - K ? ST_ISECT : ST_SEEK; break; }
        if (kp >= L) { nfl &= ~F_CAREFUL; st = ST_ISECT; break; }
        if (x < g.e) break;
        if (g.flags & SEG_LINK) {
            const U4 lk = slot_at(sl, cur + 1 + ((g.flags & SEG_WIDE) ? 1u : 0u));
            h = lk.x;
            x = lk.y;
            ncur = lk.z;
            hopped = true;
            break;
        }
        nfl &= ~F_CAREFUL;
        if (g.flags & SEG_LAST) {
            uint32_t nh = NO_HANDLE;
            if (g.flags & SEG_EDGES) {
                const U4 ed = slot_at(sl, cur + 1 + ((g.flags & SEG_WIDE) ? 1u : 0u));
                const uint32_t b = read_base(rd, kp);
                nh = sel4(b, ed.x, ed.y, ed.z, ed.w);
            }
            if (nh != NO_HANDLE) {
                h = nh;
                x = 0;
                kp -= K - 1;
                cov -= K - 1;
                nfl |= F_FRESH;
                ncur = of_cur(0u, true);
                hopped = true;
            } else st = kp > L - K ? ST_ISECT : ST_SEEK;
            break;
        }
        if (consumed >= 128u) break;
        const bool branch = (g.flags & SEG_EDGES) != 0;
        {
            if ((diff_word(dm, consumed >> 5) >> (2 * (consumed & 31u))) & 1ull) {
                uint32_t nh = NO_HANDLE;
                if (branch) {
                    const U4 ed = slot_at(sl, cur + 1 + ((g.flags & SEG_WIDE) ? 1u : 0u));
                    nh = sel4(read_base(rd, kp), ed.x, ed.y, ed.z, ed.w);
                }
                if (nh != NO_HANDLE) {
                    h = nh;
                    x = 0;
                    kp -= K - 1;
                    cov -= K - 1;
                    nfl |= F_FRESH;
                    ncur = of_cur(0u, true);
                    hopped = true;
                } else st = kp > L - K ? ST_ISECT : ST_SEEK;
                break;
            }
        }
        x += 1; kp += 1; cov += 1; consumed += 1;
        cur += 1 + ((g.flags & SEG_WIDE) ? 1u : 0u) + (branch ? 1u : 0u);
        g = seg_at(sl, cur);
        if (push_node<TRACE>(s, cols, ix, g, 64ull * s.h + x - K)) {
            restart_lists(s, K);
            return;
// ... 546 lines not shown
```

rust-pseudoaligner_amd/csrc/map_pool.hip:

```cpp
#include <hip/hip_runtime.h>

#include "kernels.hpp"
#include "lane_steps.hpp"
#include "kernel_utils.hpp"

#ifndef PA_FILL
#define PA_FILL 1
#endif
#ifndef PA_COOP_MIN
#define PA_COOP_MIN 2u
#endif
#ifndef PA_REFILL_ALIGN
#define PA_REFILL_ALIGN 1u
#endif
#ifndef PA_RARE_MIN
#define PA_RARE_MIN 16u
#endif

#ifdef PA_ISA_MARKS
#define PA_MARK(name) asm volatile("; PA_MARK " name ::: "memory")
#else
#define PA_MARK(name)
#endif

namespace pa {
namespace {

typedef __attribute__((address_space(3))) uint64_t* lds_u64;
typedef __attribute__((address_space(3))) uint32_t* lds_u32;
typedef __attribute__((address_space(3))) uint8_t* lds_u8;
typedef __attribute__((address_space(3))) uint16_t* lds_u16;
typedef __attribute__((address_space(3))) unsigned long long* lds_u64w;
typedef uint32_t u32x4 __attribute__((ext_vector_type(4)));
typedef __attribute__((address_space(3))) u32x4* lds_v4;
typedef __attribute__((address_space(1))) u32x4* glb_v4w;
typedef __attribute__((address_space(1))) const u32x4* glb_v4;
typedef __attribute__((address_space(1))) uint32_t* glb_u32w;
typedef __attribute__((address_space(1))) const uint32_t* glb_u32;
typedef __attribute__((address_space(1))) unsigned long long* glb_u64w;
__device__ __forceinline__ void store_result(glb_v4w dst, u32x4 v) {
    if (PA_NT & 2) __builtin_nontemporal_store(v, dst);
    else *dst = v;
}

typedef __attribute__((address_space(4))) const MapParams* karg_ptr;

__device__ __forceinline__ DevIndexView view_of(karg_ptr p) {
    DevIndexView v;
    v.table = p->ix.table; v.nbuckets = p->ix.nbuckets; v.blobs = p->ix.blobs; v.ledge = p->ix.ledge;
    v.seg_g = p->ix.seg_g; v.seg_nid = p->ix.seg_nid; v.ec = p->ix.ec; v.class_ref = p->ix.class_ref; v.class_len = p->ix.class_len;
    v.wtable = p->ix.wtable; v.wbuckets = p->ix.wbuckets; v.kmask = p->ix.kmask; v.kmask_hi = p->ix.kmask_hi; v.k = p->ix.k; v.num_nodes = p->ix.num_nodes; v.num_classes = p->ix.num_classes; v.num_segs = p->ix.num_segs; v.stream_nt = p->ix.stream_nt; v.bitmap_min = p->ix.bitmap_min; v.bitmap_words = p->ix.bitmap_words;
    return v;
}

constexpr uint32_t ST_NSTAT = ST_COUNT + 4;
constexpr uint32_t ST_DUAL = ST_COUNT;
constexpr uint32_t POOL_FIXED = 960;
constexpr uint32_t POOL_MAX_SLOTS = 128;
constexpr uint32_t LIST_ROW_HDR = 12;

__device__ __forceinline__ uint32_t rank_in(uint64_t m) { return __builtin_amdgcn_mbcnt_hi((uint32_t)(m >> 32), __builtin_amdgcn_mbcnt_lo((uint32_t)m, 0u)); }

__device__ __forceinline__ uint64_t shfl64(uint64_t v, uint32_t src) {
    return ((uint64_t)(uint32_t)__shfl((int)(v >> 32), (int)src, 64) << 32) | (uint32_t)__shfl((int)v, (int)src, 64);
}

__device__ __forceinline__ uint64_t arena_alloc(uint32_t cnt_alloc, uint32_t lane, karg_ptr p, lds_u64w chunk) {
    const uint32_t incl = wave_incl_scan(cnt_alloc);
    const uint32_t total = (uint32_t)__builtin_amdgcn_readlane((int)incl, 63);
    asm volatile("" ::: "memory");
    unsigned long long chunk_cur = chunk[0];
    if (total > 0) {
        if (chunk_cur + total > chunk[1]) {
            const unsigned long long want = total > PA_ARENA_CHUNK ? total : PA_ARENA_CHUNK;
            unsigned long long base = 0;
            if (lane == 0) base = atomicAdd(p->arena_top, want);
            base = ((unsigned long long)(uint32_t)__builtin_amdgcn_readfirstlane((int)(base >> 32)) << 32) | (uint32_t)__builtin_amdgcn_readfirstlane((int)base);
            chunk_cur = base;
            if (lane == 0) chunk[1] = base + want;
        }
        if (lane == 0) chunk[0] = chunk_cur + total;
    }
    asm volatile("" ::: "memory");
    return chunk_cur + (incl - cnt_alloc);
}

constexpr uint32_t NO_KEY = 0xFFFFFFFFu;
__device__ __forceinline__ void append_keys(uint32_t key, uint32_t lane, karg_ptr p, lds_u32 kchunk) {
    const uint64_t m = __ballot(key != NO_KEY);
    if (m == 0) return;
    const uint32_t cnt = (uint32_t)__popcll(m);
    const glb_u32w keys = (glb_u32w)p->keys;
    asm volatile("" ::: "memory");
    const uint32_t cur = kchunk[0], room = kchunk[1] - cur;
    uint32_t nbase = 0;
    if (cnt > room) {
        if (lane == 0) {
            nbase = (uint32_t)atomicAdd(p->keys_top, (unsigned long long)PA_KEY_CHUNK);
            if ((uint64_t)nbase + PA_KEY_CHUNK > p->keys_cap) { atomicOr(p->status, PA_STATUS_SPILL_OVERFLOW); nbase = 0; }
        }
        nbase = (uint32_t)__builtin_amdgcn_readfirstlane((int)nbase);
    }
    const uint32_t r = rank_in(m);
    if (key != NO_KEY) keys[r < room ? cur + r : nbase + (r - room)] = key;
    if (lane == 0) {
        if (cnt > room) { kchunk[0] = nbase + (cnt - room); kchunk[1] = nbase + PA_KEY_CHUNK; }
        else kchunk[0] = cur + cnt;
    }
    asm volatile("" ::: "memory");
}

__device__ __forceinline__ void append_deferred(bool has, u32x4 e0, u32x4 e1, uint32_t lane, karg_ptr p, lds_u32 dchunk) {
    const uint64_t m = __ballot(has);
    if (m == 0) return;
    const uint32_t cnt = (uint32_t)__popcll(m);
    const glb_v4w out = (glb_v4w)p->defer;
    asm volatile("" ::: "memory");
    const uint32_t cur = dchunk[0], room = dchunk[1] - cur;
    uint32_t nbase = 0;
    if (cnt > room) {
        if (lane == 0) {
            nbase = (uint32_t)atomicAdd(p->defer_top, (unsigned long long)PA_DEFER_CHUNK);
            if ((uint64_t)nbase + PA_DEFER_CHUNK > p->defer_cap) { atomicOr(p->status, PA_STATUS_SPILL_OVERFLOW); nbase = 0; }
        }
        nbase = (uint32_t)__builtin_amdgcn_readfirstlane((int)nbase);
    }
    if (has) {
        const uint32_t r = rank_in(m);
        const uint64_t at = 2ull * (r < room ? cur + r : nbase + (r - room));
        out[at] = e0;
        out[at + 1] = e1;
    }
    if (lane == 0) {
        if (cnt > room) { dchunk[0] = nbase + (cnt - room); dchunk[1] = nbase + PA_DEFER_CHUNK; }
        else dchunk[0] = cur + cnt;
    }
    asm volatile("" ::: "memory");
}

__device__ __forceinline__ uint32_t list_hits(glb_u32 ec, uint32_t xref, uint32_t nch, uint32_t maxch, const uint32_t (&b)[8]) {
    const glb_v4 xrec = (glb_v4)(ec + 4ull * xref);
    uint32_t acc = 0;
    for (uint32_t c0 = 0; c0 < maxch; c0 += 4) {
        u32x4 w[4];
#pragma unroll
        for (uint32_t t = 0; t < 4; ++t) w[t] = xrec[c0 + t < nch ? c0 + t : 0];
#pragma unroll
        for (uint32_t t = 0; t < 4; ++t)
            if (c0 + t < nch) {
                const U4 ww{w[t].x, w[t].y, w[t].z, w[t].w};
                acc |= scan_words(ww, c0 + t == 0, b);
            }
    }
    return acc;
}

__device__ __forceinline__ uint32_t wave_max(uint32_t v) {
    for (uint32_t o = 32; o; o >>= 1) v = max(v, (uint32_t)__shfl_xor((int)v, (int)o, 64));
    return (uint32_t)__builtin_amdgcn_readfirstlane((int)v);
}

__device__ __forceinline__ void window_hits(glb_u32 ec, uint32_t xref, uint32_t len, bool act, uint32_t b1, uint32_t b2, uint32_t bitmap_min, uint32_t& m1, uint32_t& m2) {
    const bool bm = act && bitmap_min != 0 && len >= bitmap_min;
    uint32_t bw[4] = {0u, 0u, 0u, 0u};
    if (__ballot(bm)) {
        if (bm) {
            const glb_u32 bits = ec + class_bitmap(xref, len);
            bw[0] = bits[b1 >> 5]; bw[1] = bits[(b1 >> 5) + 1]; bw[2] = bits[b2 >> 5]; bw[3] = bits[(b2 >> 5) + 1];
        }
    }
    act = act && !bm;
    const glb_v4 rec = (glb_v4)(ec + 4ull * xref);
    const uint32_t nch = act ? (len + 4) >> 2 : 0u;
    uint32_t c[2] = {0u, 0u}, e[2] = {nch, 0u};
    const bool lng = act && len > 64;
    if (__ballot(lng)) {
        if (lng) {
            const glb_u32 ids = ec + 4ull * xref + 1;
#pragma unroll
            for (uint32_t r = 0; r < 2; ++r) {
                const uint32_t b = r ? b2 : b1;
                uint32_t lo = 0, hi = len;
                while (lo < hi) {
                    const uint32_t mid = (lo + hi) >> 1;
                    if (ids[mid] < b) lo = mid + 1; else hi = mid;
                }
                c[r] = (1 + lo) >> 2;
                e[r] = min(nch, ((1 + lo + CLASS_WINDOW - 1) >> 2) + 1);
            }
        }
    }
    m1 = m2 = 0;
#pragma unroll
    for (uint32_t r = 0; r < 2; ++r) {
        const uint32_t mx = wave_max(e[r] > c[r] ? e[r] - c[r] : 0u);
        for (uint32_t c0 = 0; c0 < mx; c0 += 4) {
            u32x4 w[4];
#pragma unroll
            for (uint32_t t = 0; t < 4; ++t) w[t] = rec[c[r] + c0 + t < e[r] ? c[r] + c0 + t : 0u];
#pragma unroll
            for (uint32_t t = 0; t < 4; ++t)
                if (c[r] + c0 + t < e[r]) {
                    const uint32_t v[4] = {w[t].x, w[t].y, w[t].z, w[t].w};
#pragma unroll
                    for (uint32_t i = 0; i < 4; ++i) {
                        if (i == 0 && c[r] + c0 + t == 0) continue;
                        const uint32_t d1 = v[i] - b1, d2 = v[i] - b2;
                        if (d1 < CLASS_WINDOW) m1 |= 1u << d1;
                        if (d2 < CLASS_WINDOW) m2 |= 1u << d2;
                    }
                }
        }
    }
    if (bm) {
        m1 = (uint32_t)((((uint64_t)bw[1] << 32) | bw[0]) >> (b1 & 31u));
        m2 = (uint32_t)((((uint64_t)bw[3] << 32) | bw[2]) >> (b2 & 31u));
    }
}

}

namespace narrow {
#define PA_K_WIDE 0
#include "map_pool_kernel.inc"
#undef PA_K_WIDE
}

namespace wide {
#define PA_K_WIDE 1
#include "map_pool_kernel.inc"
#undef PA_K_WIDE
}

size_t pool_slot_bytes(uint32_t wpr) {
    return wpr > PA_LDS_READ_WORDS ? (size_t)wide::SLOT_FIXED_BYTES : 8 * (size_t)wpr + narrow::SLOT_FIXED_BYTES;
}
size_t pool_fixed_bytes() { return POOL_FIXED; }
uint32_t pool_max_slots() { return POOL_MAX_SLOTS; }

size_t pool_lds_bytes(uint32_t wpr, uint32_t slots) {
    const size_t wave_bytes = (POOL_FIXED + (size_t)slots * pool_slot_bytes(wpr) + 15) & ~(size_t)15;
    return wave_bytes * (PA_MAP_BLOCK / 64);
}

template <class K>
static int launch_kernel(K kernel, const MapParams& p, uint32_t grid, size_t lds_bytes, hipStream_t stream) {
    if (lds_bytes > 48 * 1024) {
        const hipError_t e = hipFuncSetAttribute(reinterpret_cast<const void*>(kernel), hipFuncAttributeMaxDynamicSharedMemorySize, (int)lds_bytes);
        if (e != hipSuccess) return (int)e;
    }
    hipLaunchKernelGGL(kernel, dim3(grid), dim3(PA_MAP_BLOCK), lds_bytes, stream, p);
    return (int)hipGetLastError();
}

int launch_map_pool(const MapParams& p, uint32_t grid, size_t lds_bytes, hipStream_t stream) {
    const bool gread = p.wpr > PA_LDS_READ_WORDS;
    if (gread) return p.trace ? launch_kernel(&wide::pa_map_pool_kernel<true, true, false, false>, p, grid, lds_bytes, stream)
                              : launch_kernel(&wide::pa_map_pool_kernel<false, true, false, false>, p, grid, lds_bytes, stream);
    if (p.trace) return launch_kernel(&narrow::pa_map_pool_kernel<true, false, false, false>, p, grid, lds_bytes, stream);
#ifdef PA_DEBUG_KNOBS
    if (p.dbg || p.ablate) return launch_kernel(&narrow::pa_map_pool_kernel<false, false, true, false>, p, grid, lds_bytes, stream);
#endif
    if (p.ix.k > 32)
        return p.pool_slots == 128 ? launch_kernel(&narrow::pa_map_pool_kernel<false, false, false, true, true>, p, grid, lds_bytes, stream)
                                   : launch_kernel(&narrow::pa_map_pool_kernel<false, false, false, false, true>, p, grid, lds_bytes, stream);
    if (p.pool_slots == 128) return launch_kernel(&narrow::pa_map_pool_kernel<false, false, false, true>, p, grid, lds_bytes, stream);
    return launch_kernel(&narrow::pa_map_pool_kernel<false, false, false, false>, p, grid, lds_bytes, stream);
}

int pool_kernel_occupancy(size_t lds_bytes, int* blocks_per_cu) {
    return (int)hipOccupancyMaxActiveBlocksPerMultiprocessor(blocks_per_cu, reinterpret_cast<const void*>(&narrow::pa_map_pool_kernel<false, false, false, false>),
                                                             PA_MAP_BLOCK, lds_bytes);
}

}
```

rust-pseudoaligner_amd/csrc/map_pool_kernel.inc:

```
namespace {

template <bool TRACE>
__device__ __forceinline__ void trace_out(const Lane& s, bool mapped, uint32_t gslot, karg_ptr p) {
    if (!TRACE) return;
    const uint32_t spill_cap = p->spill_cap;
    const uint32_t nt = l_ntrace(s);
    const uint32_t nn = mapped ? (nt < spill_cap ? nt : spill_cap) : 0;
    ((glb_u32w)p->nodes_len)[s.rid] = mapped ? nt : 0;
    const glb_u32w tr = (glb_u32w)p->trace + (uint64_t)gslot * spill_cap;
    const glb_u32w out = (glb_u32w)p->nodes_out + (uint64_t)s.rid * spill_cap;
    for (uint32_t j = 0; j < nn; ++j) out[j] = tr[j];
}

template <bool TRACE>
__device__ __forceinline__ uint32_t emit_record(Lane& s, uint32_t cnt, uint32_t cnt_alloc, uint64_t my_off, uint32_t base_len,
                                                uint32_t base_colour, uint32_t gslot, karg_ptr p, bool& defer) {
    uint32_t colour = NO_CLASS, class_off = (uint32_t)my_off;
    bool novel = false;
    if (my_off + cnt_alloc > p->arena_cap) atomicOr(p->status, PA_STATUS_ARENA_FULL);
    if (cnt == base_len) {
        colour = base_colour;
        class_off = PA_CLASS_REF | base_colour;
    } else novel = cnt != 0;
    if (l_flags(s) & F_SPILL_OVERFLOW) atomicOr(p->status, PA_STATUS_SPILL_OVERFLOW);
    ((glb_v4w)p->results)[s.rid] = u32x4{l_cov(s), l_mism(s) | PA_MAPPED_BIT, class_off, cnt};
    trace_out<TRACE>(s, true, gslot, p);
    const glb_u32w colour_out = (glb_u32w)p->colour_out;
    if (novel && (p->keys != nullptr || colour_out != nullptr) && my_off + cnt_alloc <= p->arena_cap) {
        defer = true;
        s.lk = 0;
        return NO_KEY;
    }
    if (colour_out) colour_out[s.rid] = colour;
    s.lk = 0;
    const uint32_t num_classes = p->ix.num_classes;
    return cnt == 0 ? num_classes + 1 : colour == NO_CLASS ? num_classes : colour;
}

__device__ __forceinline__ uint32_t queue_of(Lane& s, uint32_t K) {
    uint32_t st = l_st(s);
    if (st == ST_ISECT) {
        const uint32_t fl = l_flags(s);
        if (!(fl & F_LISTS)) {
            const uint32_t todo = window_todo(s);
            if (todo == 2) { restart_lists(s, K); return ST_SEEK; }
            st = todo ? ST_F_MASK : ST_F_BITS;
        } else st = l_ncol(s) <= 3 ? ST_F_LIGHT : (fl & F_SMALL_BASE) ? ST_F_SCAN : ST_F_COOP;
        l_set_st(s, st);
    }
    return st == ST_NONE ? (uint32_t)ST_F_BITS : st;
}

template <bool GREAD>
__device__ __forceinline__ void refill_slot(Lane& s, uint64_t rid, uint32_t slot, karg_ptr p, lds_u64 rd, lds_u32 wc, uint32_t S, uint32_t wpr,
                                            uint32_t K) {
    const uint32_t* lens = p->lens;
    uint32_t L = lens ? lens[rid] : p->uniform_len;
    if (L > wpr * 32) L = wpr * 32;
    if (!GREAD) {
        const uint64_t* src = p->tiles + ((rid >> 6) * wpr) * 64 + (rid & 63);
        if (wpr == 5) {
            const bool nt = (PA_NT & 1) || p->ix.stream_nt;
            const uint64_t v0 = ld_stream(src, nt), v1 = ld_stream(src + 64, nt), v2 = ld_stream(src + 128, nt), v3 = ld_stream(src + 192, nt), v4 = ld_stream(src + 256, nt);
            rd[slot] = v0; rd[S + slot] = v1; rd[2 * S + slot] = v2; rd[3 * S + slot] = v3; rd[4 * S + slot] = v4;
        } else if (wpr == 4) {
            const bool nt = (PA_NT & 1) || p->ix.stream_nt;
            const uint64_t v0 = ld_stream(src, nt), v1 = ld_stream(src + 64, nt), v2 = ld_stream(src + 128, nt), v3 = ld_stream(src + 192, nt);
            rd[slot] = v0; rd[S + slot] = v1; rd[2 * S + slot] = v2; rd[3 * S + slot] = v3;
        } else
        for (uint32_t w0 = 0; w0 < wpr; w0 += 8) {
            uint64_t v[8];
#pragma unroll
            for (uint32_t i = 0; i < 8; ++i) v[i] = w0 + i < wpr ? PA_LD(1, src + (uint64_t)(w0 + i) * 64) : 0ull;
#pragma unroll
            for (uint32_t i = 0; i < 8; ++i)
                if (w0 + i < wpr) rd[(w0 + i) * S + slot] = v[i];
        }
    }
    lane_start(s, (uint32_t)rid, L, K);
    wc[2 * slot + 1] = (uint32_t)rid;
}

__device__ __forceinline__ void lane_load(Lane& s, lds_v4 stA, lds_v4 stB, lds_v4 stC, uint32_t slot) {
    const u32x4 a = stA[slot], b = stB[slot];
    s.lk = a.x; s.cm = a.y; s.h = a.z; s.of = a.w; s.rr = b.x; s.rm = b.y; s.ph = b.z; s.nc = b.w;
#if PA_K_WIDE
    const u32x4 c = stC[slot];
    s.xl = c.x; s.xm = c.y; s.xt = c.z;
#else
    (void)stC;
#endif
}
__device__ __forceinline__ void lane_store(const Lane& s, lds_v4 stA, lds_v4 stB, lds_v4 stC, uint32_t slot) {
    stA[slot] = u32x4{s.lk, s.cm, s.h, s.of};
    stB[slot] = u32x4{s.rr, s.rm, s.ph, s.nc};
#if PA_K_WIDE
    stC[slot] = u32x4{s.xl, s.xm, s.xt, 0u};
#else
    (void)stC;
#endif
}
constexpr uint32_t SLOT_FIXED_BYTES = 32 + 16 + 8 + (PA_K_WIDE ? 16 : 0);

}

#ifndef PA_MAP_MIN_BLOCKS
#define PA_MAP_MIN_BLOCKS 3
#endif
template <bool TRACE, bool GREAD, bool DBG, bool S128 = false, bool KBIG = false>
__global__ __launch_bounds__(PA_MAP_BLOCK, PA_MAP_MIN_BLOCKS) void pa_map_pool_kernel(const MapParams p_arg) {
    karg_ptr kp = (karg_ptr)__builtin_amdgcn_kernarg_segment_ptr();
    (void)p_arg;
#define p (*kp)
#define PA_DBG (DBG && p.dbg)
#define PA_ABLATE(bit) (DBG && (p.ablate & (bit)))
    extern __shared__ __attribute__((aligned(16))) uint8_t smem[];
    const uint32_t lane = lane_id();
    const uint32_t wave_in_block = (uint32_t)__builtin_amdgcn_readfirstlane((int)(threadIdx.x >> 6));
    const uint32_t waves_per_block = PA_MAP_BLOCK / 64;
    const uint32_t wave = blockIdx.x * waves_per_block + wave_in_block;
    const uint32_t nwaves = gridDim.x * waves_per_block;
    const uint32_t S = S128 ? 128u : p.pool_slots, wpr = p.wpr;
    const uint32_t lwpr = GREAD ? 0u : wpr;

    const uint32_t wave_bytes = (POOL_FIXED + S * (8 * lwpr + SLOT_FIXED_BYTES) + 15) & ~15u;
    uint8_t* const wbase = smem + wave_in_block * wave_bytes;
    const lds_u64w chunk = (lds_u64w)wbase;
    const lds_u32 dbg = (lds_u32)(wbase + 16);
    const lds_u64w dbg_clk = (lds_u64w)(wbase + 16 + 8 * ST_NSTAT);
    const lds_u32 kchunk = (lds_u32)(wbase + 256);
    const lds_u32 dchunk = (lds_u32)(wbase + 264);
    const lds_u64 rd = (lds_u64)(wbase + POOL_FIXED);
    const lds_v4 stA = (lds_v4)(wbase + POOL_FIXED + 8 * lwpr * S);
    const lds_v4 stB = (lds_v4)(wbase + POOL_FIXED + (8 * lwpr + 16) * S);
    constexpr uint32_t XW = PA_K_WIDE ? 16u : 0u;
    const lds_v4 stC = (lds_v4)(wbase + POOL_FIXED + (8 * lwpr + 32) * S);
    const lds_v4 win = (lds_v4)(wbase + POOL_FIXED + (8 * lwpr + 32 + XW) * S);
    const lds_u32 wc = (lds_u32)(wbase + POOL_FIXED + (8 * lwpr + 48 + XW) * S);
    const lds_u8 sb = (lds_u8)(wbase + 768);
    const lds_u8 poplist = (lds_u8)(wbase + 896);
    if (lane < 64) ((lds_u32)wbase)[lane] = 0;
    if (lane < 4) kchunk[lane] = 0;
    ((lds_u16)sb)[lane] = (uint16_t)((lane < S ? (uint32_t)ST_EMPTY : 0xFFu) | ((lane + 64 < S ? (uint32_t)ST_EMPTY : 0xFFu) << 8));

    const uint32_t ntiles = (uint32_t)((p.n_reads + 63) >> 6);
    const uint32_t chunk_tiles = ntiles / (nwaves * 4) >= 16 ? 16u : ntiles / (nwaves * 4) >= 1 ? ntiles / (nwaves * 4) : 1u;
    uint64_t next = (uint64_t)wave * chunk_tiles << 6;
    uint64_t end = (uint64_t)(wave + 1) * chunk_tiles << 6;
    if (end > p.n_reads) end = p.n_reads;
    if (next > end) next = end;
    bool more = true;
    uint32_t seen = nwaves * chunk_tiles;

    const bool counting = p.keys != nullptr;

#define PA_CNT(t) ((uint32_t)__popcll(__ballot(st_lo == (t))) + (uint32_t)__popcll(__ballot(st_hi == (t))))
#define PA_POP(t, nn, out)                                                                         \
    {                                                                                              \
        const uint64_t m0_ = __ballot(st_lo == (t)), m1_ = __ballot(st_hi == (t));                 \
        const uint32_t r1_ = (uint32_t)__popcll(m0_) + rank_in(m1_);                               \
        if (st_lo == (t)) poplist[rank_in(m0_)] = (uint8_t)lane;                                   \
        if (st_hi == (t) && r1_ < 64) poplist[r1_] = (uint8_t)(lane + 64);                         \
        asm volatile("" ::: "memory");                                                             \
        out = lane < (nn) ? (uint32_t)poplist[lane] : 0u;                                          \
        asm volatile("" ::: "memory");                                                             \
    }

    for (;;) {
        PA_MARK("loop_top");
        asm volatile("" : "+s"(kp) : : "memory");
        const DevIndexView ix = view_of(kp);
        const glb_u32 ec = (glb_u32)ix.ec;
        const uint32_t K = ix.k, allowed = p.allowed, spill_cap = p.spill_cap;
        if (next == end && more) {
            const uint32_t share = (ntiles > seen ? ntiles - seen : 0u) / (2 * nwaves);
            const uint32_t take = share >= 16 ? 16u : share >= 2 ? share : 2u;
            uint32_t t0 = 0;
            if (lane == 0) t0 = atomicAdd(p.tile_ctr, take);
            t0 = (uint32_t)__builtin_amdgcn_readfirstlane((int)t0) + nwaves * chunk_tiles;
            seen = t0 + take;
            if (t0 >= ntiles) more = false;
            else {
                next = (uint64_t)t0 << 6;
                end = (uint64_t)(t0 + take) << 6;
                if (end > p.n_reads) end = p.n_reads;
            }
        }
        const uint32_t st2 = (uint32_t)((lds_u16)sb)[lane];
        const uint32_t st_lo = st2 & 0xFFu, st_hi = st2 >> 8;
        const uint64_t left = end - next;
        const uint32_t nempty = PA_CNT(ST_EMPTY);
        const uint32_t nrefill = (uint32_t)(left < (uint64_t)nempty ? left : (uint64_t)nempty);
        uint32_t best = 0, sel = ST_EMPTY;
        uint32_t bestn = 0;
#define PA_CONSIDER(t, c) { const uint32_t c_ = (c); if (best < 64 && c_ > best) { best = c_; bestn = c_; sel = (t); } }
#define PA_CONSIDER_RARE_MIN(t, c, mn) { const uint32_t c_ = (c), w_ = (PA_RARE_MIN && c_ >= (mn)) ? 64u + c_ : c_; \
                                         if (best < 64 && w_ > best) { best = w_; bestn = c_; sel = (t); } }
#define PA_CONSIDER_RARE(t, c) PA_CONSIDER_RARE_MIN(t, c, PA_RARE_MIN)
        constexpr uint32_t RARE = (1u << ST_LEFT) | (1u << ST_F_LIGHT) | (1u << ST_F_SCAN) | (1u << ST_F_COOP) | (1u << ST_F_MASK);
        const bool any_rare = __ballot((((RARE >> (st_lo & 31u)) | (RARE >> (st_hi & 31u))) & 1u) != 0) != 0;
        const uint32_t n_bits_q = PA_CNT(ST_F_BITS), n_seek_q = PA_CNT(ST_SEEK), n_fwd_q = PA_CNT(ST_FWD);
        if (any_rare) {
            PA_CONSIDER_RARE_MIN(ST_F_COOP, PA_CNT(ST_F_COOP), PA_COOP_MIN)
            PA_CONSIDER_RARE(ST_F_SCAN, PA_CNT(ST_F_SCAN))
            PA_CONSIDER_RARE(ST_F_LIGHT, PA_CNT(ST_F_LIGHT))
            PA_CONSIDER_RARE(ST_F_MASK, PA_CNT(ST_F_MASK))
            PA_CONSIDER(ST_F_BITS, n_bits_q)
            PA_CONSIDER(ST_FWD, n_fwd_q)
            PA_CONSIDER_RARE(ST_LEFT, PA_CNT(ST_LEFT))
            PA_CONSIDER(ST_SEEK, n_seek_q)
            PA_CONSIDER(ST_EMPTY, nrefill)
        } else {
            const uint32_t cb = min(n_bits_q, 64u), cf = min(n_fwd_q, 64u), cs = min(n_seek_q, 64u), ce = min(nrefill, 64u);
            best = max(max(cb, cf), max(cs, ce));
            sel = cb == best ? (uint32_t)ST_F_BITS : cf == best ? (uint32_t)ST_FWD : cs == best ? (uint32_t)ST_SEEK : (uint32_t)ST_EMPTY;
            bestn = cb == best ? n_bits_q : cf == best ? n_fwd_q : cs == best ? n_seek_q : nrefill;
        }
#undef PA_CONSIDER
#undef PA_CONSIDER_RARE
#undef PA_CONSIDER_RARE_MIN
        if (best == 0) break;
#ifndef PA_SEEK_MIN
#define PA_SEEK_MIN 32u
#endif
        const bool seek_ok = n_seek_q >= PA_SEEK_MIN || n_fwd_q < 24;
        const bool dual = (sel == ST_FWD || sel == ST_SEEK) && (K <= 32 || KBIG) && n_seek_q != 0 && n_fwd_q != 0 && seek_ok && !PA_ABLATE(4u);
        if (dual) sel = ST_FWD;
        uint32_t n_own = dual ? (n_fwd_q < 64 ? n_fwd_q : 64) : bestn < 64 ? bestn : 64;
        if (PA_REFILL_ALIGN > 1 && sel == ST_EMPTY && n_own >= PA_REFILL_ALIGN && (uint64_t)n_own < left) n_own &= ~(PA_REFILL_ALIGN - 1u);
        const uint32_t n_fill = (PA_FILL && sel == ST_F_BITS && left != 0) ? (64 - n_own < nempty ? 64 - n_own : nempty) : 0u;
        const uint32_t n = n_own + n_fill;
        const uint32_t n2 = dual ? (n_seek_q < 64 ? n_seek_q : 64) : 0u;
        if (PA_DBG && lane == 0) {
            dbg[dual ? ST_DUAL : sel] += 1;
            dbg[ST_NSTAT + (dual ? ST_DUAL : sel)] += n + n2;
        }
        const unsigned long long t_sec = PA_DBG ? __builtin_readcyclecounter() : 0ull;

        PA_MARK("picked");
        const bool active = lane < n;
        uint32_t slot, slot2 = 0;
        PA_POP(sel, n_own, slot)
        if (n_fill) {
            uint32_t eslot;
            PA_POP((uint32_t)ST_EMPTY, n_fill, eslot)
            const uint32_t mine = (uint32_t)__shfl((int)eslot, (int)((lane - n_own) & 63u), 64);
            if (lane >= n_own && active) slot = mine;
        }
        const bool active2 = lane < n2;
        if (dual) PA_POP((uint32_t)ST_SEEK, n2, slot2)
        const uint32_t gslot = wave * S + slot;
        Lane s;
        {
            lane_load(s, stA, stB, stC, slot);
            s.rid = wc[2 * slot + 1];
            if (n_fill && lane >= n_own) s.lk = 0;
        }
        const ReadRef rr = GREAD ? ReadRef{p.tiles + ((uint64_t)(s.rid >> 6) * wpr) * 64 + (s.rid & 63), 64u, wpr} : ReadRef{(const uint64_t*)(rd + slot), S, wpr, true};
        const glb_u32w row = (glb_u32w)p.spill + (uint64_t)gslot * spill_cap;
        const ColRef cols{(uint32_t*)&win[slot], (uint32_t*)(wc + 2 * slot), (uint32_t*)row, (uint32_t*)(row + 4), (uint32_t*)(row + 8),
                          (uint32_t*)(row + LIST_ROW_HDR), spill_cap - LIST_ROW_HDR, (uint32_t*)row,
                          TRACE ? (uint32_t*)((glb_u32w)p.trace + (uint64_t)gslot * spill_cap) : nullptr};

        uint32_t nq2 = 0xFFu;
        PA_MARK("popped");
        const unsigned long long t_pop = PA_DBG ? __builtin_readcyclecounter() : 0ull;
        if (sel == ST_EMPTY) {
            if (active) refill_slot<GREAD>(s, next + lane, slot, kp, rd, wc, S, wpr, K);
            next += n;
        } else if (sel == ST_SEEK) {
            if (active) seek_step(s, ix, rr);
        } else if (sel == ST_FWD) {
            __builtin_amdgcn_s_waitcnt(0x0F70);
            Lane s2;
            {
#if PA_K_WIDE
                lane_load(s2, stA, stB, stC, slot2);
                if (!active2) l_zero(s2);
#else
                const u32x4 a = stA[slot2], b = stB[slot2];
                s2.lk = active2 ? a.x : 0u; s2.cm = active2 ? a.y : 0u; s2.h = active2 ? a.z : 0u; s2.of = active2 ? a.w : 0u;
                s2.rr = active2 ? b.x : 0u; s2.rm = active2 ? b.y : 0u; s2.ph = active2 ? b.z : 0u; s2.nc = active2 ? b.w : 0u;
#endif
                s2.rid = 0;
            }
            if (!active) l_zero(s);
            const uint32_t rid2 = GREAD && active2 ? wc[2 * slot2 + 1] : 0u;
            const ReadRef rr2 = GREAD ? ReadRef{p.tiles + ((uint64_t)(rid2 >> 6) * wpr) * 64 + (rid2 & 63), 64u, wpr} : ReadRef{(const uint64_t*)(rd + slot2), S, wpr};
            SeekProbe pq;
            FwdLoad fl;
            PA_MARK("dual_state2");
            pq.klo = pq.khi = pq.pending = 0; pq.v = U4{0u, 0u, NO_HANDLE, 0u};
            SeekProbe2 pq2;
            if (KBIG) {
                pq2.k0 = pq2.v0 = pq2.k1 = pq2.v1 = U4{0u, 0u, 0u, 0u}; pq2.v0.x = pq2.v1.x = NO_HANDLE; pq2.w0 = pq2.w1 = pq2.w2 = pq2.w3 = 0;
                if (n2) seek_issue_k2(s2, ix, rr2, pq2);
            }
            if (!KBIG && n2) seek_issue(s2, ix, rr2, pq);
            const bool two_l = !KBIG && active2 && seek_two(s2, K);
            const bool pairs = __popcll(__ballot(two_l)) >= 8;
            const bool two = two_l && pairs;
            SeekProbe pq1;
            pq1.klo = pq1.khi = pq1.pending = 0; pq1.v = U4{0u, 0u, NO_HANDLE, 0u};
            if (pairs) seek_issue(s2, ix, rr2, pq1, PA_SEEK_STRIDE, two);
            fwd_issue(s, ix, fl);
            __builtin_amdgcn_sched_barrier(0);
            PA_MARK("dual_issued");
            if (active2) {
                if (KBIG) seek_complete_k2(s2, K, pq2);
                else seek_complete2(s2, K, pq, two, pq1);
                nq2 = queue_of(s2, K);
                lane_store(s2, stA, stB, stC, slot2);
            }
            __builtin_amdgcn_sched_barrier(0);
            const unsigned long long t1 = PA_DBG ? __builtin_readcyclecounter() : 0ull;
            PA_MARK("dual_second");
            if (active) fwd_finish<TRACE>(s, ix, rr, cols, allowed, fl);
            PA_MARK("dual_fwd_done");
            if (PA_DBG && lane == 0) {
                const unsigned long long t3 = __builtin_readcyclecounter();
                dbg[ST_COUNT + 1] += 1; dbg[ST_COUNT + 3] += 1;
                dbg_clk[ST_COUNT + 1] += t1 - t_pop; dbg_clk[ST_COUNT + 3] += t3 - t1;
            }
            PA_MARK("dual_seek_done");
        } else if (sel == ST_LEFT) {
            if (active) left_step<TRACE>(s, ix, rr, cols, allowed);
        } else if (sel == ST_F_BITS) {
            PA_MARK("bits_begin");
            uint32_t ckey = NO_KEY;
            bool dfr = false;
            u32x4 d0{0u, 0u, 0u, 0u}, d1{0u, 0u, 0u, 0u};
            if (active && lane < n_own) {
                const bool mapped = l_st(s) != ST_NONE;
                const u32x4 w = win[slot];
                const uint32_t cand = wc[2 * slot];
                const uint32_t count = mapped ? (uint32_t)(__popc(w.y) + __popc(w.w)) : 0u;
                if (mapped && count != 0 && cand == NO_CLASS) {
                    dfr = true;
                    d0 = u32x4{s.rid, l_cov(s), l_mism(s), PA_DEFER_WINDOW | count};
                    d1 = w;
                    trace_out<TRACE>(s, true, gslot, kp);
                    s.lk = 0;
                } else {
                    const bool is_ref = mapped && count != 0;
                    if (!PA_ABLATE(1u))
                        store_result((glb_v4w)p.results + s.rid, mapped ? u32x4{l_cov(s), l_mism(s) | PA_MAPPED_BIT, is_ref ? PA_CLASS_REF | cand : 0u, count}
                                                                        : u32x4{0u, 0u, 0u, 0u});
                    trace_out<TRACE>(s, mapped, gslot, kp);
                    const glb_u32w colour_out = (glb_u32w)p.colour_out;
                    if (colour_out) colour_out[s.rid] = is_ref ? cand : NO_CLASS;
                    ckey = !mapped ? ix.num_classes + 2 : count == 0 ? ix.num_classes + 1 : cand;
                    s.lk = 0;
                }
            }
            {
                const uint64_t freed = __ballot(active && s.lk == 0);
                const uint32_t nfree = (uint32_t)__popcll(freed);
                uint32_t take = (uint32_t)(left < (uint64_t)nfree ? left : (uint64_t)nfree);
                if (PA_REFILL_ALIGN > 1 && take >= PA_REFILL_ALIGN && (uint64_t)take < left) take &= ~(PA_REFILL_ALIGN - 1u);
                if (take && !PA_ABLATE(8u)) {
                    if (active && s.lk == 0 && rank_in(freed) < take) refill_slot<GREAD>(s, next + rank_in(freed), slot, kp, rd, wc, S, wpr, K);
                    next += take;
                }
            }
            if (counting && !PA_ABLATE(2u)) append_keys(ckey, lane, kp, kchunk);
            append_deferred(dfr, d0, d1, lane, kp, dchunk);
            PA_MARK("bits_end");
        } else if (sel == ST_F_MASK) {
            const u32x4 w = active ? win[slot] : u32x4{0u, 0u, 0u, 0u};
            const uint32_t np_mine = active ? l_npend(s) : 0u;
            uint32_t a1 = w.y, a2 = w.w;
            for (uint64_t todo = __ballot(active && np_mine <= 64); todo;) {
                const uint32_t want = ((todo >> lane) & 1ull) ? np_mine : 0u;
                const uint32_t incl = wave_incl_scan(want);
                const uint32_t start = incl - want;
                const bool inpass = want != 0 && incl <= 64;
                const uint64_t pass = __ballot(inpass);
                todo &= ~pass;
                uint32_t Lr = 64, jg = 0, seg_end = 0;
                for (uint64_t m = pass; m; m &= m - 1) {
                    const uint32_t o = (uint32_t)(__ffsll((unsigned long long)m) - 1);
                    const uint32_t st = (uint32_t)__builtin_amdgcn_readlane((int)start, (int)o);
                    const uint32_t nc = (uint32_t)__builtin_amdgcn_readlane((int)np_mine, (int)o);
                    if (lane - st < nc) { Lr = o; jg = lane - st; seg_end = st + nc; }
                }
                const bool gact = Lr < 64;
                const int src = (int)(Lr & 63u);
                const uint32_t b1 = (uint32_t)__shfl((int)w.x, src, 64), b2 = (uint32_t)__shfl((int)w.z, src, 64), slotL = (uint32_t)__shfl((int)slot, src, 64);
                const glb_u32w rowL = (glb_u32w)p.spill + (uint64_t)(wave * S + slotL) * spill_cap;
                uint32_t xref = 0, xlen = 0;
                if (gact) { xref = rowL[2 * jg]; xlen = rowL[2 * jg + 1]; }
                uint32_t m1, m2;
                window_hits(ec, xref, xlen, gact, b1, b2, ix.bitmap_min, m1, m2);
                for (uint32_t o = 1; o < 64; o <<= 1) {
                    const uint32_t t1 = (uint32_t)__shfl_down((int)m1, o, 64), t2 = (uint32_t)__shfl_down((int)m2, o, 64);
                    if (gact && lane + o < seg_end) { m1 &= t1; m2 &= t2; }
                }
                const uint32_t r1 = (uint32_t)__shfl((int)m1, (int)(start & 63u), 64), r2 = (uint32_t)__shfl((int)m2, (int)(start & 63u), 64);
                if (inpass) { a1 &= r1; a2 &= r2; }
            }
            for (uint64_t todo = __ballot(active && np_mine > 64); todo; todo &= todo - 1) {
                const uint32_t Lr = (uint32_t)(__ffsll((unsigned long long)todo) - 1);
                const uint32_t b1 = (uint32_t)__shfl((int)w.x, (int)Lr, 64), b2 = (uint32_t)__shfl((int)w.z, (int)Lr, 64);
                const uint32_t npL = (uint32_t)__shfl((int)np_mine, (int)Lr, 64), slotL = (uint32_t)__shfl((int)slot, (int)Lr, 64);
                const glb_u32w rowL = (glb_u32w)p.spill + (uint64_t)(wave * S + slotL) * spill_cap;
                uint32_t r1 = 0xFFFFFFFFu, r2 = 0xFFFFFFFFu;
                for (uint32_t g = 0; g < npL; g += 64) {
                    const uint32_t ci = g + lane;
                    const bool gact = ci < npL;
                    uint32_t xref = 0, xlen = 0;
                    if (gact) { xref = rowL[2 * ci]; xlen = rowL[2 * ci + 1]; }
                    uint32_t m1, m2;
                    window_hits(ec, xref, xlen, gact, b1, b2, ix.bitmap_min, m1, m2);
                    if (gact) { r1 &= m1; r2 &= m2; }
                }
                for (uint32_t o = 32; o; o >>= 1) {
                    r1 &= (uint32_t)__shfl_xor((int)r1, (int)o, 64);
                    r2 &= (uint32_t)__shfl_xor((int)r2, (int)o, 64);
                }
                if (lane == Lr) { a1 &= r1; a2 &= r2; }
            }
            if (active) {
                if (a1 != w.y || a2 != w.w) wc[2 * slot] = NO_CLASS;
                win[slot] = u32x4{w.x, a1, w.z, a2};
                s.nc = (s.nc & ~NC_COL_MASK) | 1u;
                l_set_st(s, ST_F_BITS);
            }
        } else if (sel == ST_F_SCAN) {
            Isect is;
            is.base_len = is.base_ref = is.base_colour = 0;
            if (active) isect_pick(s, cols, is);
            const uint32_t ncol_mine = l_ncol(s);
            if (active && ncol_mine > 3) is.base_colour = ec[4ull * is.base_ref];
            uint32_t my_alive = 0;
            for (uint64_t todo = __ballot(active && ncol_mine > 0 && ncol_mine <= 64); todo;) {
                const uint32_t want = ((todo >> lane) & 1ull) ? ncol_mine : 0u;
                const uint32_t incl = wave_incl_scan(want);
                const uint32_t start = incl - want;
                const bool inpass = want != 0 && incl <= 64;
                const uint64_t pass = __ballot(inpass);
                todo &= ~pass;
                uint32_t Lr = 64, jg = 0;
                for (uint64_t m = pass; m; m &= m - 1) {
                    const uint32_t o = (uint32_t)(__ffsll((unsigned long long)m) - 1);
                    const uint32_t st = (uint32_t)__builtin_amdgcn_readlane((int)start, (int)o);
                    const uint32_t nc = (uint32_t)__builtin_amdgcn_readlane((int)ncol_mine, (int)o);
                    if (lane - st < nc) { Lr = o; jg = lane - st; }
                }
                const bool gact = Lr < 64;
                const int src = (int)(Lr & 63u);
                const uint32_t bref = (uint32_t)__shfl((int)is.base_ref, src, 64), blen = (uint32_t)__shfl((int)is.base_len, src, 64),
                               slotL = (uint32_t)__shfl((int)slot, src, 64);
                const glb_u32w rowL = (glb_u32w)p.spill + (uint64_t)(wave * S + slotL) * spill_cap;
                const glb_v4 brec = (glb_v4)(ec + 4ull * bref);
                const u32x4 q0 = brec[0], q1 = brec[1], q2 = brec[2];
                const uint32_t b[8] = {q0.y, q0.z, q0.w, q1.x, q1.y, q1.z, q1.w, blen > 7 ? q2.x : 0xFFFFFFFFu};
                uint32_t xref = bref, xlen = 0;
                if (gact) {
                    if (jg < LDS_CLASSES) { xref = rowL[jg]; xlen = rowL[4 + jg]; }
                    else { const u32x4 qd = *(glb_v4)(rowL + LIST_ROW_HDR + 4 * (jg - LDS_CLASSES)); xref = qd.x; xlen = qd.y; }
                }
                const bool mine = xref != bref;
                const uint32_t nch = mine ? (xlen + 4) >> 2 : 0u;
// ... 221 lines not shown
```

Before: 13.27 billion reads/s.

## Add compact 8-byte dictionary slots with tagged k-mer hi bits for K<=25

Introduces a compact hash-table format for k<=25 in which each slot is one 64-bit word. The word packs the k-mer's high bits plus bucket-derived tag bits, a displacement counter, the chain handle, the offset and the flags, in place of the 16-byte four-word slot. Host and device insert and find paths, the seek probe evaluation and the pool kernel are templated on the format, and the compact variant is dispatched when it fits. This halves the table footprint and the bytes touched per probe on the memory-bound lookup path. The cost is extra bit manipulation per probe and a more complex, riskier encoding, plus new verification hooks.

```diff
diff --git a/rust-pseudoaligner_amd/csrc/device_flatten.cpp b/rust-pseudoaligner_amd/csrc/device_flatten.cpp
--- a/rust-pseudoaligner_amd/csrc/device_flatten.cpp
+++ b/rust-pseudoaligner_amd/csrc/device_flatten.cpp
@@ -36,6 +36,9 @@
     v.stream_nt = 0;
     v.bitmap_min = bitmap_min;
     v.bitmap_words = bitmap_words;
+    v.dict_compact = dict_fmt.compact;
+    v.dict_w = dict_fmt.tag_w;
+    v.dict_hbits = dict_fmt.hbits;
     return v;
 }
 
@@ -100,6 +103,8 @@
 struct HostAtomics {
     static bool cas(uint32_t* p, uint32_t expect, uint32_t v) { return __atomic_compare_exchange_n(p, &expect, v, false, __ATOMIC_RELAXED, __ATOMIC_RELAXED); }
     static void and_(uint32_t* p, uint32_t m) { __atomic_fetch_and(p, m, __ATOMIC_RELAXED); }
+    static uint64_t cas64(uint64_t* p, uint64_t expect, uint64_t v) { __atomic_compare_exchange_n(p, &expect, v, false, __ATOMIC_RELAXED, __ATOMIC_RELAXED); return expect; }
+    static void and64(uint64_t* p, uint64_t m) { __atomic_fetch_and(p, m, __ATOMIC_RELAXED); }
 };
 
 template <>
@@ -108,15 +113,18 @@
     static constexpr uint32_t SLOTS = SLOTS_PER_BUCKET;
     uint32_t* words;
     uint64_t nbuckets;
-    void insert_mt(uint64_t kmer, uint32_t handle, uint32_t off) { dict_insert_home<HostAtomics>(words, (uint32_t)nbuckets, kmer, handle, off); }
-    void insert_rest_mt(uint64_t kmer, uint32_t handle, uint32_t off) { dict_insert_rest<HostAtomics>(words, (uint32_t)nbuckets, kmer, handle, off); }
+    DictFormat fmt;
+    void insert_mt(uint64_t kmer, uint32_t handle, uint32_t off) { dict_insert_home<HostAtomics>(words, (uint32_t)nbuckets, fmt, kmer, handle, off); }
+    void insert_rest_mt(uint64_t kmer, uint32_t handle, uint32_t off) { dict_insert_rest<HostAtomics>(words, (uint32_t)nbuckets, fmt, kmer, handle, off); }
     bool find(uint64_t kmer, uint32_t& handle, uint32_t& off, uint32_t* probes_out = nullptr) const {
         uint32_t probes = 0;
-        const bool found = dict_find64(words, (uint32_t)nbuckets, kmer, handle, off, probes);
+        const bool found = dict_find64(words, (uint32_t)nbuckets, fmt, kmer, handle, off, probes);
         if (probes_out) *probes_out = probes;
         return found;
     }
 };
+
+std::atomic<uint64_t> g_last_dict[4];
 
 }
 
@@ -519,7 +527,7 @@
             fn(km, blk, dict_entry_off(c, o == 0, block_slot_of(out.blobs.data() + (uint64_t)blk * CH_BLOCK, (c & (CH_STRIDE - 1)) + k - 1)));
         }
     };
-    Dict<KT> dict{nullptr, 0};
+    Dict<KT> dict{};
     if (device_dict) {
         out.node_kcum.resize((size_t)N + 1);
         out.node_kcum[0] = 0;
@@ -530,28 +538,62 @@
     for (double load = load0; !device_dict; load *= 0.75) {
         out.nbuckets = std::max<uint64_t>(1, (uint64_t)((double)nk / (Dict<KT>::SLOTS * load)) + 1);
         if (out.nbuckets >= 0xFFFFFFFFull) return fail(PA_ERR_UNSUPPORTED, "dictionary exceeds 2^32 buckets");
-        out.table.assign(out.nbuckets * BUCKET_WORDS, 0xFFFFFFFFu);
-        dict = Dict<KT>{out.table.data(), out.nbuckets};
+        out.dict_fmt = sizeof(KT) == 8 ? dict_format(k, out.nbuckets, out.blobs.size() / CH_BLOCK) : DictFormat{0u, 0u, 0u};
+        out.table.assign(out.nbuckets * dict_bucket_words(out.dict_fmt), 0xFFFFFFFFu);
+        dict = Dict<KT>{};
+        dict.words = out.table.data();
+        dict.nbuckets = out.nbuckets;
+        if constexpr (sizeof(KT) == 8) dict.fmt = out.dict_fmt;
         par_ranges(threads, N, [&](uint64_t a, uint64_t b, int) {
             for (uint64_t i = a; i < b; ++i) node_kmers((uint32_t)i, [&](KT km, uint32_t h, uint32_t o) { dict.insert_mt(km, h, o); });
         });
         par_ranges(threads, N, [&](uint64_t a, uint64_t b, int) {
             for (uint64_t i = a; i < b; ++i) node_kmers((uint32_t)i, [&](KT km, uint32_t h, uint32_t o) { dict.insert_rest_mt(km, h, o); });
         });
-        std::atomic<uint32_t> bad{NO_HANDLE}, far{0};
+        std::atomic<uint32_t> bad{NO_HANDLE}, far{0}, maxd{0};
+        std::atomic<uint64_t> moved{0}, moved2{0};
         par_ranges(threads, N, [&](uint64_t a, uint64_t b, int) {
+            uint32_t md = 0;
+            uint64_t m1 = 0, m2 = 0;
             for (uint64_t i = a; i < b; ++i)
                 node_kmers((uint32_t)i, [&](KT km, uint32_t h, uint32_t o) {
                     uint32_t fh, fo, probes = 0;
                     if (!dict.find(km, fh, fo, &probes) || fh != h || fo != o) bad.store((uint32_t)i);
                     if (probes > DICT_MAX_PROBES) far.store(1);
+                    md = std::max(md, probes); m1 += probes >= 1; m2 += probes >= 2;
                 });
+            moved += m1; moved2 += m2;
+            for (uint32_t c = maxd.load(); md > c && !maxd.compare_exchange_weak(c, md);) {}
         });
+        if (far.load()) continue;
         if (bad.load() != NO_HANDLE) return fail(PA_ERR_FORMAT, "a k-mer of node %u occurs twice in the graph", bad.load());
-        if (!far.load()) break;
+        g_last_dict[0] = 4 * dict_bucket_words(out.dict_fmt) / Dict<KT>::SLOTS; g_last_dict[1] = maxd.load(); g_last_dict[2] = moved.load(); g_last_dict[3] = moved2.load();
+        break;
     }
     return PA_OK;
 }
+
+}
+
+extern "C" {
+int pa_dict_slot_layout(uint32_t k, uint64_t nbuckets, uint64_t blocks, uint32_t out[4]) {
+    const pa::DictFormat f = pa::dict_format(k, nbuckets, blocks);
+    out[0] = f.compact; out[1] = f.tag_w; out[2] = f.hbits; out[3] = f.compact ? pa::CS_HANDLE_SHIFT + f.hbits : 0u;
+    return f.compact ? 8 : 16;
+}
+void pa_dict_tags(const uint64_t* kmers, uint64_t n, uint32_t nbuckets, uint32_t w, uint32_t d, uint32_t* bucket, uint64_t* tag) {
+    for (uint64_t i = 0; i < n; ++i) {
+        uint32_t home, x;
+        bucket[i] = pa::pa_bucket_home_x(kmers[i], nbuckets, home, x);
+        tag[i] = pa::cs_tag_d(kmers[i], x, d, w);
+    }
+}
+void pa_dict_last_build(uint64_t out[4]) {
+    for (int i = 0; i < 4; ++i) out[i] = pa::g_last_dict[i].load();
+}
+}
+
+namespace pa {
 
 int flatten_for_device(const pa_flat_index& f, int threads, FlatDevice& out, bool device_dict) {
     if (f.k < PA_MIN_K || f.k > PA_MAX_K) return fail(PA_ERR_UNSUPPORTED, "k=%u outside [%u,%u]", f.k, PA_MIN_K, PA_MAX_K);
diff --git a/rust-pseudoaligner_amd/csrc/device_flatten.hpp b/rust-pseudoaligner_amd/csrc/device_flatten.hpp
--- a/rust-pseudoaligner_amd/csrc/device_flatten.hpp
+++ b/rust-pseudoaligner_amd/csrc/device_flatten.hpp
@@ -11,6 +11,7 @@
 struct FlatDevice {
     std::vector<uint32_t> table;
     uint64_t nbuckets = 0;
+    DictFormat dict_fmt{0u, 0u, 0u};
     std::vector<uint8_t> blobs;
     std::vector<uint32_t> handle;
     std::vector<uint32_t> node_s;
@@ -33,7 +34,7 @@
 int flatten_for_device(const pa_flat_index& f, int threads, FlatDevice& out, bool device_dict = false);
 
 #ifdef __HIPCC__
-int device_fill_index(const FlatDevice& fd, const uint8_t* d_blobs, DeviceBuffer<uint32_t>& table, uint64_t* nbuckets);
+int device_fill_index(const FlatDevice& fd, const uint8_t* d_blobs, DeviceBuffer<uint32_t>& table, uint64_t* nbuckets, DictFormat* fmt);
 #endif
 
 }
diff --git a/rust-pseudoaligner_amd/csrc/device_index.hip b/rust-pseudoaligner_amd/csrc/device_index.hip
--- a/rust-pseudoaligner_amd/csrc/device_index.hip
+++ b/rust-pseudoaligner_amd/csrc/device_index.hip
@@ -9,6 +9,7 @@
 #include <thread>
 
 #include "device_flatten.hpp"
+#include "dict_slots.hpp"
 #include "hip_buffer.hpp"
 #include "kernels.hpp"
 #include "lane_steps.hpp"
@@ -258,7 +259,7 @@
     if (idx->num_cus <= 0) idx->num_cus = 256;
     rc = upload(idx->d_blobs, fd.blobs);
     if (rc == PA_OK) rc = upload(idx->d_ledge, fd.ledge);
-    if (rc == PA_OK) rc = device_fill_index(fd, idx->d_blobs.get(), idx->d_table, &fd.nbuckets);
+    if (rc == PA_OK) rc = device_fill_index(fd, idx->d_blobs.get(), idx->d_table, &fd.nbuckets, &fd.dict_fmt);
     if (rc == PA_OK) rc = upload(idx->d_seg_g, fd.seg_g);
     if (rc == PA_OK) rc = upload(idx->d_seg_nid, fd.seg_nid);
     if (rc == PA_OK) rc = upload(idx->d_ec, fd.ec);
@@ -281,11 +282,12 @@
     idx->dv.class_ref = idx->d_class_ref.get();
     idx->dv.class_len = idx->d_class_len.get();
     idx->dv.wtable = idx->d_wtable.get();
-    idx->dv.stream_nt = (fd.k <= 32 && fd.nbuckets * BUCKET_WORDS * 4 > (512ull << 20)) ? 1u : 0u;
+    const uint64_t bytes_table = fd.nbuckets * dict_bucket_words(fd.dict_fmt) * 4;
+    idx->dv.stream_nt = (fd.k <= 32 && bytes_table > (512ull << 20)) ? 1u : 0u;
     pa_index_stats& s = idx->stats;
     s.num_kmers = fd.num_kmers;
     s.table_slots = fd.nbuckets * SLOTS_PER_BUCKET;
-    s.bytes_table = fd.nbuckets * BUCKET_WORDS * 4;
+    s.bytes_table = bytes_table;
     s.bytes_graph = fd.blobs.size() + fd.ledge.size() * 4 + fd.seg_g.size() * 12;
     s.bytes_classes = (fd.ec.size() + fd.class_ref.size() + fd.class_len.size() + ctab.size() + fd.wtable.size()) * 4;
     s.bytes_total = s.bytes_table + s.bytes_graph + s.bytes_classes;
@@ -294,6 +296,39 @@
     s.k = fd.k;
     s.max_class_len = fd.max_class_len;
     *out = idx;
+    return PA_OK;
+}
+
+extern "C" int pa_index_dict_check(const pa_index* idx, const pa_flat_index* flat, uint64_t out[6]) {
+    if (!idx || !flat || !out) return fail(PA_ERR_INVALID_ARG, "null argument");
+    if (flat->k > 32) return fail(PA_ERR_UNSUPPORTED, "one-word dictionaries only");
+    int rc = use_device(idx->device);
+    if (rc != PA_OK) return rc;
+    FlatDevice fd;
+    rc = flatten_for_device(*flat, std::max(1, usable_threads()), fd, false);
+    if (rc != PA_OK) return rc;
+    const DictFormat gfmt{idx->dv.dict_compact, idx->dv.dict_w, idx->dv.dict_hbits};
+    std::vector<uint32_t> gtable(idx->dv.nbuckets * dict_bucket_words(gfmt));
+    PA_HIP_TRY(hipMemcpy(gtable.data(), idx->dv.table, gtable.size() * 4, hipMemcpyDeviceToHost));
+    const uint32_t k = fd.k;
+    const uint64_t mask = k >= 32 ? ~0ull : ((1ull << (2 * k)) - 1);
+    uint64_t n = 0, bad = 0;
+    for (uint32_t i = 0; i < fd.num_nodes; ++i)
+        for (uint32_t o = 0; o + k <= flat->node_len[i]; ++o, ++n) {
+            const uint32_t c = fd.node_s[i] + o, blk = fd.handle[i] + (c >> CH_STRIDE_LOG2), rel = c & (CH_STRIDE - 1);
+            uint64_t w[5];
+            memcpy(w, fd.blobs.data() + (uint64_t)blk * CH_BLOCK + CH_SEQ_BYTES, 32);
+            w[4] = 0;
+            const uint32_t wi = rel >> 5, sh = (rel & 31) * 2;
+            const uint64_t km = (sh ? (w[wi] >> sh) | (w[wi + 1] << (64 - sh)) : w[wi]) & mask;
+            uint32_t h0 = 0, o0 = 0, p0 = 0, h1 = 0, o1 = 0, p1 = 0;
+            const bool f0 = dict_find64(fd.table.data(), (uint32_t)fd.nbuckets, fd.dict_fmt, km, h0, o0, p0);
+            const bool f1 = dict_find64(gtable.data(), (uint32_t)idx->dv.nbuckets, gfmt, km, h1, o1, p1);
+            if (!f0 || !f1 || h0 != h1 || o0 != o1 || h0 != blk) ++bad;
+        }
+    out[0] = n; out[1] = bad;
+    out[2] = 4 * dict_bucket_words(fd.dict_fmt) / SLOTS_PER_BUCKET; out[3] = 4 * dict_bucket_words(gfmt) / SLOTS_PER_BUCKET;
+    out[4] = fd.nbuckets; out[5] = idx->dv.nbuckets;
     return PA_OK;
 }
 
diff --git a/rust-pseudoaligner_amd/csrc/device_layout.hpp b/rust-pseudoaligner_amd/csrc/device_layout.hpp
--- a/rust-pseudoaligner_amd/csrc/device_layout.hpp
+++ b/rust-pseudoaligner_amd/csrc/device_layout.hpp
@@ -45,6 +45,44 @@
 constexpr uint32_t SLOT_FLAG_OVERFLOW = 8u;
 constexpr double DICT_LOAD = 0.25;
 constexpr uint32_t DICT_MAX_PROBES = 15;
+constexpr uint32_t CS_WORDS = 2, CS_BUCKET_WORDS = 8;
+constexpr uint32_t CS_FLAG_MASK = 15u;
+constexpr uint32_t CS_OFF_SHIFT = 4, CS_OFF_BITS = 11, CS_OFF_MASK = (1u << CS_OFF_BITS) - 1u;
+constexpr uint32_t CS_HANDLE_SHIFT = CS_OFF_SHIFT + CS_OFF_BITS;
+constexpr uint32_t CS_D_BITS = 4;
+constexpr uint32_t CS_MAX_K = 25;
+
+struct DictFormat {
+    uint32_t compact;
+    uint32_t tag_w;
+    uint32_t hbits;
+};
+PA_HD uint32_t ceil_log2_u64(uint64_t v) {
+    uint32_t n = 0;
+    while (n < 63 && (1ull << n) < v) ++n;
+    return n;
+}
+PA_HD DictFormat dict_format(uint32_t k, uint64_t nbuckets, uint64_t blocks) {
+    DictFormat f{0u, 0u, 0u};
+    if (k > CS_MAX_K || nbuckets == 0 || nbuckets > 0xFFFFFFFFull) return f;
+    const uint32_t hi_bits = k > 16 ? 2 * k - 32 : 0u;
+    const uint32_t w = ceil_log2_u64(((1ull << 32) + nbuckets - 1) / nbuckets);
+    const uint32_t h = ceil_log2_u64(blocks + 2);
+    if (h > 31 || hi_bits + w + CS_D_BITS + h + CS_HANDLE_SHIFT > 64) return f;
+    f.compact = 1u; f.tag_w = w; f.hbits = h;
+    return f;
+}
+PA_HD uint32_t dict_bucket_words(const DictFormat& f) { return f.compact ? CS_BUCKET_WORDS : BUCKET_WORDS; }
+PA_HD uint64_t cs_tag_d(uint64_t kmer, uint32_t x, uint32_t d, uint32_t w) {
+    const uint64_t tag = ((kmer >> 32) << w) | ((uint64_t)x & ((1ull << w) - 1ull));
+    return (tag << CS_D_BITS) | d;
+}
+PA_HD uint64_t cs_expect(uint64_t kmer, uint32_t x, uint32_t d, uint32_t w, uint32_t hbits) { return cs_tag_d(kmer, x, d, w) << (CS_HANDLE_SHIFT + hbits); }
+PA_HD uint32_t cs_handle(uint64_t v, uint32_t hbits) { return (uint32_t)(v >> CS_HANDLE_SHIFT) & ((1u << hbits) - 1u); }
+PA_HD bool cs_empty(uint64_t v, uint32_t hbits) { return cs_handle(v, hbits) == (1u << hbits) - 1u; }
+PA_HD bool cs_holds(uint64_t v, uint64_t expect, uint32_t hbits) { return !cs_empty(v, hbits) && ((v ^ expect) >> (CS_HANDLE_SHIFT + hbits)) == 0; }
+PA_HD uint32_t cs_off(uint64_t v) { return ((uint32_t)v >> CS_OFF_SHIFT) & CS_OFF_MASK; }
+PA_HD uint32_t cs_flags(uint64_t v) { return ~(uint32_t)v & CS_FLAG_MASK; }
 
 struct alignas(16) U4 {
     uint32_t x, y, z, w;
@@ -75,6 +113,9 @@
     uint32_t stream_nt;
     uint32_t bitmap_min;
     uint32_t bitmap_words;
+    uint32_t dict_compact;
+    uint32_t dict_w;
+    uint32_t dict_hbits;
 };
 
 PA_HD uint32_t class_record_chunks(uint32_t len) { return len < 4 ? 2u : (len + 4) >> 2; }
diff --git a/rust-pseudoaligner_amd/csrc/dict_slots.hpp b/rust-pseudoaligner_amd/csrc/dict_slots.hpp
--- a/rust-pseudoaligner_amd/csrc/dict_slots.hpp
+++ b/rust-pseudoaligner_amd/csrc/dict_slots.hpp
@@ -11,18 +11,48 @@
     A::and_(slot + 3, off | ~SLOT_OFF_MASK);
     return true;
 }
-
 template <class A>
-PA_HD void dict_insert_home(uint32_t* table, uint32_t nbuckets, uint64_t km, uint32_t handle, uint32_t off) {
-    uint32_t home;
-    const uint32_t b = pa_bucket_home(km, nbuckets, home);
-    slot_claim<A>(table + (uint64_t)b * BUCKET_WORDS + SLOT_WORDS * home, km, handle, off);
+PA_HD bool cslot_claim(uint64_t* slot, uint64_t body, uint32_t hbits) {
+    uint64_t cur = ~0ull;
+    for (;;) {
+        const uint64_t seen = A::cas64(slot, cur, body | (cur & CS_FLAG_MASK));
+        if (seen == cur) return true;
+        if (!cs_empty(seen, hbits)) return false;
+        cur = seen;
+    }
+}
+PA_HD uint64_t cslot_body(uint64_t km, uint32_t x, uint32_t d, uint32_t handle, uint32_t off, const DictFormat& fmt) {
+    return cs_expect(km, x, d & ((1u << CS_D_BITS) - 1u), fmt.tag_w, fmt.hbits) | ((uint64_t)handle << CS_HANDLE_SHIFT) | ((uint64_t)off << CS_OFF_SHIFT);
 }
 
 template <class A>
-PA_HD void dict_insert_rest(uint32_t* table, uint32_t nbuckets, uint64_t km, uint32_t handle, uint32_t off) {
-    uint32_t home;
-    uint32_t b = pa_bucket_home(km, nbuckets, home);
+PA_HD void dict_insert_home(uint32_t* table, uint32_t nbuckets, const DictFormat& fmt, uint64_t km, uint32_t handle, uint32_t off) {
+    uint32_t home, x;
+    const uint32_t b = pa_bucket_home_x(km, nbuckets, home, x);
+    if (fmt.compact) cslot_claim<A>(reinterpret_cast<uint64_t*>(table) + (uint64_t)b * SLOTS_PER_BUCKET + home, cslot_body(km, x, 0, handle, off, fmt), fmt.hbits);
+    else slot_claim<A>(table + (uint64_t)b * BUCKET_WORDS + SLOT_WORDS * home, km, handle, off);
+}
+
+template <class A>
+PA_HD void dict_insert_rest(uint32_t* table, uint32_t nbuckets, const DictFormat& fmt, uint64_t km, uint32_t handle, uint32_t off) {
+    uint32_t home, x;
+    uint32_t b = pa_bucket_home_x(km, nbuckets, home, x);
+    if (fmt.compact) {
+        uint64_t* t64 = reinterpret_cast<uint64_t*>(table);
+        if (cs_holds(t64[(uint64_t)b * SLOTS_PER_BUCKET + home], cs_expect(km, x, 0, fmt.tag_w, fmt.hbits), fmt.hbits)) return;
+        for (uint32_t d = 0;; ++d) {
+            uint64_t* line = t64 + (uint64_t)b * SLOTS_PER_BUCKET;
+            uint64_t* hs = line + home;
+            if (d && cslot_claim<A>(hs, cslot_body(km, x, d, handle, off, fmt), fmt.hbits)) return;
+            for (uint32_t i = 0; i < 3; ++i)
+                if (cslot_claim<A>(line + ((home + 1 + i) & 3u), cslot_body(km, x, d, handle, off, fmt), fmt.hbits)) {
+                    A::and64(hs, ~(uint64_t)(1u << i));
+                    return;
+                }
+            A::and64(hs, ~(uint64_t)SLOT_FLAG_OVERFLOW);
+            if (++b == nbuckets) b = 0;
+        }
+    }
     {
         const uint32_t* hs = table + (uint64_t)b * BUCKET_WORDS + SLOT_WORDS * home;
         if (hs[2] != NO_HANDLE && hs[0] == (uint32_t)km && hs[1] == (uint32_t)(km >> 32)) return;
@@ -41,9 +71,26 @@
     }
 }
 
-PA_HD bool dict_find64(const uint32_t* table, uint32_t nbuckets, uint64_t km, uint32_t& handle, uint32_t& off, uint32_t& probes) {
-    uint32_t home;
-    uint32_t b = pa_bucket_home(km, nbuckets, home);
+PA_HD bool dict_find64(const uint32_t* table, uint32_t nbuckets, const DictFormat& fmt, uint64_t km, uint32_t& handle, uint32_t& off, uint32_t& probes) {
+    uint32_t home, x;
+    uint32_t b = pa_bucket_home_x(km, nbuckets, home, x);
+    if (fmt.compact) {
+        const uint64_t* t64 = reinterpret_cast<const uint64_t*>(table);
+        for (probes = 0; probes < nbuckets; ++probes) {
+            const uint64_t* line = t64 + (uint64_t)b * SLOTS_PER_BUCKET;
+            const uint64_t e = cs_expect(km, x, probes & ((1u << CS_D_BITS) - 1u), fmt.tag_w, fmt.hbits);
+            const uint64_t v = line[home];
+            if (cs_holds(v, e, fmt.hbits)) { handle = cs_handle(v, fmt.hbits); off = cs_off(v); return true; }
+            const uint32_t fl = cs_flags(v);
+            for (uint32_t c = fl & 7u; c; c &= c - 1) {
+                const uint64_t v2 = line[(home + 1 + pa_ctz32(c)) & 3u];
+                if (cs_holds(v2, e, fmt.hbits)) { handle = cs_handle(v2, fmt.hbits); off = cs_off(v2); return true; }
+            }
+            if (!(fl & SLOT_FLAG_OVERFLOW)) return false;
+            if (++b == nbuckets) b = 0;
+        }
+        return false;
+    }
     const uint32_t klo = (uint32_t)km, khi = (uint32_t)(km >> 32);
     for (probes = 0; probes < nbuckets; ++probes) {
         const uint32_t* line = table + (uint64_t)b * BUCKET_WORDS;
diff --git a/rust-pseudoaligner_amd/csrc/index_fill.hip b/rust-pseudoaligner_amd/csrc/index_fill.hip
--- a/rust-pseudoaligner_amd/csrc/index_fill.hip
+++ b/rust-pseudoaligner_amd/csrc/index_fill.hip
@@ -27,6 +27,8 @@
 struct DeviceAtomics {
     __device__ static bool cas(uint32_t* p, uint32_t expect, uint32_t v) { return atomicCAS(p, expect, v) == expect; }
     __device__ static void and_(uint32_t* p, uint32_t m) { atomicAnd(p, m); }
+    __device__ static uint64_t cas64(uint64_t* p, uint64_t expect, uint64_t v) { return atomicCAS(reinterpret_cast<unsigned long long*>(p), (unsigned long long)expect, (unsigned long long)v); }
+    __device__ static void and64(uint64_t* p, uint64_t m) { atomicAnd(reinterpret_cast<unsigned long long*>(p), (unsigned long long)m); }
 };
 template <> struct FillOps<u128> {
     static constexpr uint32_t SLOTS = 2;
@@ -62,13 +64,13 @@
 };
 
 template <class KT>
-__device__ __forceinline__ bool dict_find(const uint32_t* table, uint32_t nbuckets, KT km, uint32_t& handle, uint32_t& off, uint32_t& probes);
+__device__ __forceinline__ bool dict_find(const uint32_t* table, uint32_t nbuckets, const DictFormat& fmt, KT km, uint32_t& handle, uint32_t& off, uint32_t& probes);
 template <>
-__device__ __forceinline__ bool dict_find<uint64_t>(const uint32_t* table, uint32_t nbuckets, uint64_t km, uint32_t& handle, uint32_t& off, uint32_t& probes) {
-    return dict_find64(table, nbuckets, km, handle, off, probes);
+__device__ __forceinline__ bool dict_find<uint64_t>(const uint32_t* table, uint32_t nbuckets, const DictFormat& fmt, uint64_t km, uint32_t& handle, uint32_t& off, uint32_t& probes) {
+    return dict_find64(table, nbuckets, fmt, km, handle, off, probes);
 }
 template <>
-__device__ __forceinline__ bool dict_find<u128>(const uint32_t* table, uint32_t nbuckets, u128 km, uint32_t& handle, uint32_t& off, uint32_t& probes) {
+__device__ __forceinline__ bool dict_find<u128>(const uint32_t* table, uint32_t nbuckets, const DictFormat&, u128 km, uint32_t& handle, uint32_t& off, uint32_t& probes) {
     uint32_t b = FillOps<u128>::bucket(km, nbuckets);
     for (probes = 0; probes < nbuckets; ++probes) {
         const int r = FillOps<u128>::look(table + (uint64_t)b * BUCKET_WORDS, km, handle, off);
@@ -107,14 +109,14 @@
 template <class KT>
 __global__ __launch_bounds__(256) void pa_fill_insert_kernel(const uint8_t* __restrict__ blobs, const uint32_t* __restrict__ handle, const uint32_t* __restrict__ node_s,
                                                              const uint64_t* __restrict__ kcum, uint32_t num_nodes, uint64_t nk, uint32_t k, uint32_t* table,
-                                                             uint32_t nbuckets, int pass) {
+                                                             uint32_t nbuckets, DictFormat fmt, int pass) {
     const uint64_t g = (uint64_t)blockIdx.x * blockDim.x + threadIdx.x;
     if (g >= nk) return;
     const KmerAt a = kmer_at(blobs, handle, node_s, kcum, num_nodes, g, k);
     const KT km = FillOps<KT>::get(a.seq, a.rel, k);
     if constexpr (sizeof(KT) == 8) {
-        if (pass == 0) dict_insert_home<DeviceAtomics>(table, nbuckets, km, a.block, a.off);
-        else dict_insert_rest<DeviceAtomics>(table, nbuckets, km, a.block, a.off);
+        if (pass == 0) dict_insert_home<DeviceAtomics>(table, nbuckets, fmt, km, a.block, a.off);
+        else dict_insert_rest<DeviceAtomics>(table, nbuckets, fmt, km, a.block, a.off);
     } else {
         if (pass != 0) return;
         uint32_t b = FillOps<KT>::bucket(km, nbuckets);
@@ -128,18 +130,18 @@
 template <class KT>
 __global__ __launch_bounds__(256) void pa_fill_verify_kernel(const uint8_t* __restrict__ blobs, const uint32_t* __restrict__ handle, const uint32_t* __restrict__ node_s,
                                                              const uint64_t* __restrict__ kcum, uint32_t num_nodes, uint64_t nk, uint32_t k,
-                                                             const uint32_t* __restrict__ table, uint32_t nbuckets, uint32_t* __restrict__ flags) {
+                                                             const uint32_t* __restrict__ table, uint32_t nbuckets, DictFormat fmt, uint32_t* __restrict__ flags) {
     const uint64_t g = (uint64_t)blockIdx.x * blockDim.x + threadIdx.x;
     if (g >= nk) return;
     const KmerAt a = kmer_at(blobs, handle, node_s, kcum, num_nodes, g, k);
     const KT km = FillOps<KT>::get(a.seq, a.rel, k);
     uint32_t fh = 0, fo = 0, probes = 0;
-    if (!dict_find<KT>(table, nbuckets, km, fh, fo, probes) || fh != a.block || fo != a.off) atomicMin(flags, a.node);
+    if (!dict_find<KT>(table, nbuckets, fmt, km, fh, fo, probes) || fh != a.block || fo != a.off) atomicMin(flags, a.node);
     if (probes > DICT_MAX_PROBES) flags[1] = 1;
 }
 
 template <class KT>
-int fill_t(const FlatDevice& fd, const uint8_t* d_blobs, DeviceBuffer<uint32_t>& table_out, uint64_t* nbuckets_out) {
+int fill_t(const FlatDevice& fd, const uint8_t* d_blobs, DeviceBuffer<uint32_t>& table_out, uint64_t* nbuckets_out, DictFormat* fmt_out) {
     const uint32_t N = fd.num_nodes, k = fd.k;
     const uint64_t nk = fd.num_kmers;
     DeviceBuffer<uint32_t> table, d_handle, d_node_s, d_flags;
@@ -153,45 +155,53 @@
     if (N) PA_HIP_TRY(hipMemcpy(d_node_s.get(), fd.node_s.data(), (size_t)N * 4, hipMemcpyHostToDevice));
     PA_HIP_TRY(hipMemcpy(d_kcum.get(), fd.node_kcum.data(), ((size_t)N + 1) * 8, hipMemcpyHostToDevice));
     uint64_t nbuckets = 0;
+    const uint64_t blocks = fd.blobs.size() / CH_BLOCK;
+    auto format_of = [&](uint64_t nb) { return sizeof(KT) == 8 ? dict_format(k, nb, blocks) : DictFormat{0u, 0u, 0u}; };
+    DictFormat fmt{0u, 0u, 0u};
     double load0 = FillOps<KT>::LOAD;
     {
         size_t free_b = 0, total_b = 0;
         const double dense = sizeof(KT) == 8 ? 0.5 : FillOps<KT>::LOAD;
-        if (load0 < dense && hipMemGetInfo(&free_b, &total_b) == hipSuccess && (double)nk / (FillOps<KT>::SLOTS * load0) * BUCKET_WORDS * 4 > (double)free_b / 4) load0 = dense;
+        const double nb0 = (double)nk / (FillOps<KT>::SLOTS * load0);
+        if (load0 < dense && hipMemGetInfo(&free_b, &total_b) == hipSuccess && nb0 * dict_bucket_words(format_of((uint64_t)nb0 + 1)) * 4 > (double)free_b / 4) load0 = dense;
     }
     if (const char* v = knob_str("PA_DICT_LOAD")) { const double x = atof(v); if (x > 0.01 && x <= 0.95) load0 = x; }
     for (double load = load0;; load *= 0.75) {
         nbuckets = std::max<uint64_t>(1, (uint64_t)((double)nk / (FillOps<KT>::SLOTS * load)) + 1);
         if (nbuckets >= 0xFFFFFFFFull) return fail(PA_ERR_UNSUPPORTED, "dictionary exceeds 2^32 buckets");
-        if ((e = table.alloc(nbuckets * BUCKET_WORDS)) != PA_OK) return e;
-        PA_HIP_TRY(hipMemsetAsync(table.get(), 0xFF, nbuckets * BUCKET_WORDS * 4, nullptr));
+        fmt = format_of(nbuckets);
+        const uint64_t table_words = nbuckets * dict_bucket_words(fmt);
+        if ((e = table.alloc(table_words)) != PA_OK) return e;
+        PA_HIP_TRY(hipMemsetAsync(table.get(), 0xFF, table_words * 4, nullptr));
         const uint32_t init[4] = {NO_HANDLE, 0u, NO_HANDLE, NO_HANDLE};
         PA_HIP_TRY(hipMemcpy(d_flags.get(), init, 16, hipMemcpyHostToDevice));
         if (nk) {
             const dim3 grid((uint32_t)((nk + 255) / 256));
             for (int pass = 0; pass < (sizeof(KT) == 8 ? 2 : 1); ++pass) {
                 hipLaunchKernelGGL(pa_fill_insert_kernel<KT>, grid, dim3(256), 0, nullptr, d_blobs, d_handle.get(), d_node_s.get(), d_kcum.get(), N, nk, k,
-                                   table.get(), (uint32_t)nbuckets, pass);
+                                   table.get(), (uint32_t)nbuckets, fmt, pass);
                 PA_HIP_TRY(hipGetLastError());
             }
             hipLaunchKernelGGL(pa_fill_verify_kernel<KT>, grid, dim3(256), 0, nullptr, d_blobs, d_handle.get(), d_node_s.get(), d_kcum.get(), N, nk, k,
-                               table.get(), (uint32_t)nbuckets, d_flags.get());
+                               table.get(), (uint32_t)nbuckets, fmt, d_flags.get());
             PA_HIP_TRY(hipGetLastError());
         }
         uint32_t flags[4];
         PA_HIP_TRY(hipMemcpy(flags, d_flags.get(), 16, hipMemcpyDeviceToHost));
+        if (flags[1]) continue;
         if (flags[0] != NO_HANDLE) return fail(PA_ERR_FORMAT, "a k-mer of node %u occurs twice in the graph", flags[0]);
-        if (!flags[1]) break;
+        break;
     }
     *nbuckets_out = nbuckets;
+    *fmt_out = fmt;
     table_out = std::move(table);
     return PA_OK;
 }
 
 }
 
-int device_fill_index(const FlatDevice& fd, const uint8_t* d_blobs, DeviceBuffer<uint32_t>& table, uint64_t* nbuckets) {
-    return fd.k <= 32 ? fill_t<uint64_t>(fd, d_blobs, table, nbuckets) : fill_t<u128>(fd, d_blobs, table, nbuckets);
-}
-
-}
+int device_fill_index(const FlatDevice& fd, const uint8_t* d_blobs, DeviceBuffer<uint32_t>& table, uint64_t* nbuckets, DictFormat* fmt) {
+    return fd.k <= 32 ? fill_t<uint64_t>(fd, d_blobs, table, nbuckets, fmt) : fill_t<u128>(fd, d_blobs, table, nbuckets, fmt);
+}
+
+}
diff --git a/rust-pseudoaligner_amd/csrc/lane_steps_body.hpp b/rust-pseudoaligner_amd/csrc/lane_steps_body.hpp
--- a/rust-pseudoaligner_amd/csrc/lane_steps_body.hpp
+++ b/rust-pseudoaligner_amd/csrc/lane_steps_body.hpp
@@ -464,37 +464,60 @@
     uint32_t klo, khi;
     uint32_t pending;
 };
+template <int FMT>
+PA_HD bool seek_compact(const DevIndexView& ix) { return FMT == 2 ? ix.dict_compact != 0 : FMT == 1; }
+template <int FMT>
+PA_HD void seek_none(SeekProbe& q) {
+    q.klo = q.khi = q.pending = 0;
+    q.v = FMT == 0 ? U4{0u, 0u, NO_HANDLE, 0u} : U4{NO_HANDLE, NO_HANDLE, NO_HANDLE, NO_HANDLE};
+}
 struct SeekProbe2 {
     U4 k0, v0, k1, v1;
     uint32_t w0, w1, w2, w3;
 };
 constexpr uint32_t SK_NAMED = 7u, SK_FULL = 8u, SK_MASK = 15u;
-PA_HD uint32_t pa_bucket_home(uint64_t kmer, uint32_t nbuckets, uint32_t& home) {
+PA_HD uint32_t pa_bucket_home_x(uint64_t kmer, uint32_t nbuckets, uint32_t& home, uint32_t& x_out) {
     uint32_t x = (uint32_t)kmer * 0x9E3779B1u + (uint32_t)(kmer >> 32) * 0x85EBCA77u;
     x ^= x >> 15;
     x *= 0x2C1B3C6Du;
     x ^= x >> 13;
     home = x & 3u;
+    x_out = x;
 #if defined(__HIP_DEVICE_COMPILE__)
     return __umulhi(x, nbuckets);
 #else
     return (uint32_t)(((uint64_t)x * nbuckets) >> 32);
 #endif
 }
+PA_HD uint32_t pa_bucket_home(uint64_t kmer, uint32_t nbuckets, uint32_t& home) {
+    uint32_t x;
+    return pa_bucket_home_x(kmer, nbuckets, home, x);
+}
 #endif
 #if PA_LS_LANE
 PA_HD bool seek_two(const Lane& s, uint32_t K) { return (l_flags(s) & F_SPEC) && l_probe(s) == 0 && l_kp(s) + PA_SEEK_STRIDE <= l_L(s) - K; }
 PA_HD uint32_t l_pending(const Lane& s) { return s.rm & SK_MASK; }
+template <int FMT = 2>
 PA_HD void seek_issue(const Lane& s, const DevIndexView& ix, ReadRef rd, SeekProbe& q, uint32_t ahead = 0, bool live = true) {
     const uint32_t at = live ? l_kp(s) + ahead : l_kp(s);
     const uint64_t kmer = read_window_in(rd, at) & ix.kmask;
-    uint32_t home;
-    uint32_t b = pa_bucket_home(kmer, (uint32_t)ix.nbuckets, home) + (ahead ? 0u : l_probe(s));
+    uint32_t home, x;
+    const uint32_t probe = ahead ? 0u : l_probe(s);
+    uint32_t b = pa_bucket_home_x(kmer, (uint32_t)ix.nbuckets, home, x) + probe;
     if (b >= (uint32_t)ix.nbuckets) b -= (uint32_t)ix.nbuckets;
     q.pending = ahead ? 0u : l_pending(s);
     const uint32_t named = q.pending & SK_NAMED;
     uint32_t slot = named ? (home + 1u + pa_ctz32(named)) & 3u : home;
     if (!live) { b = 0; slot = 0; }
+    if (seek_compact<FMT>(ix)) {
+        const uint64_t v = ld_stream(reinterpret_cast<const uint64_t*>(ix.table) + (uint64_t)b * SLOTS_PER_BUCKET + slot, (PA_NT & 4) || ix.stream_nt);
+        const uint64_t e = cs_expect(kmer, x, probe, ix.dict_w, ix.dict_hbits);
+        q.v.x = (uint32_t)v;
+        q.v.y = (uint32_t)(v >> 32);
+        q.klo = (uint32_t)e;
+        q.khi = (uint32_t)(e >> 32);
+        return;
+    }
     q.v = ld_stream(reinterpret_cast<const U4*>(ix.table + (uint64_t)b * BUCKET_WORDS + SLOT_WORDS * slot), (PA_NT & 4) || ix.stream_nt);
     q.klo = (uint32_t)kmer;
     q.khi = (uint32_t)(kmer >> 32);
@@ -508,22 +531,35 @@
 PA_HD void seek_finish(Lane& s, uint32_t K, uint32_t h, uint32_t off, bool full, uint32_t probe);
 #endif
 #if PA_LS_COMMON
-PA_HD void seek_eval(const SeekProbe& q, uint32_t& h, uint32_t& off, bool& full, uint32_t& pending) {
+template <int FMT = 2>
+PA_HD void seek_eval(const SeekProbe& q, const DevIndexView& ix, uint32_t& h, uint32_t& off, bool& full, uint32_t& pending) {
     h = NO_HANDLE;
     off = 0;
-    const bool hit = slot_holds(q.v, q.klo, q.khi);
-    if (hit) { h = q.v.z; off = q.v.w & SLOT_OFF_MASK; }
+    bool hit;
+    uint32_t flags;
+    if (seek_compact<FMT>(ix)) {
+        const uint64_t v = ((uint64_t)q.v.y << 32) | q.v.x, e = ((uint64_t)q.khi << 32) | q.klo;
+        hit = cs_holds(v, e, ix.dict_hbits);
+        if (hit) { h = cs_handle(v, ix.dict_hbits); off = cs_off(v); }
+        flags = cs_flags(v);
+    } else {
+        hit = slot_holds(q.v, q.klo, q.khi);
+        if (hit) { h = q.v.z; off = q.v.w & SLOT_OFF_MASK; }
+        flags = slot_flags(q.v);
+    }
     const uint32_t named = q.pending & SK_NAMED;
-    const uint32_t next = named ? (named & (named - 1u)) | (q.pending & SK_FULL) : slot_flags(q.v);
+    const uint32_t next = named ? (named & (named - 1u)) | (q.pending & SK_FULL) : flags;
     pending = hit ? 0u : (next & SK_NAMED) ? next : 0u;
     full = (next & SK_FULL) != 0;
 }
 #endif
 #if PA_LS_LANE
-PA_HD bool seek_settle(Lane& s, uint32_t K, const SeekProbe& q, bool more) {
+template <int FMT = 2>
+PA_HD bool seek_settle(Lane& s, const DevIndexView& ix, const SeekProbe& q, bool more) {
+    const uint32_t K = ix.k;
     uint32_t h, off, pending;
     bool full;
-    seek_eval(q, h, off, full, pending);
+    seek_eval<FMT>(q, ix, h, off, full, pending);
     if (pending) { s.rm = (s.rm & ~SK_MASK) | pending; return true; }
     const uint32_t probe = l_probe(s);
     if (!more || h != NO_HANDLE || (full && probe < DICT_MAX_PROBES)) {
@@ -535,10 +571,12 @@
     s.nc &= ~(15u << NC_PROBE_SHIFT);
     return false;
 }
-PA_HD void seek_complete(Lane& s, uint32_t K, const SeekProbe& q) { (void)seek_settle(s, K, q, false); }
-PA_HD void seek_complete2(Lane& s, uint32_t K, const SeekProbe& q0, bool two, const SeekProbe& q1) {
-    if (seek_settle(s, K, q0, two)) return;
-    (void)seek_settle(s, K, q1, false);
+template <int FMT = 2>
+PA_HD void seek_complete(Lane& s, const DevIndexView& ix, const SeekProbe& q) { (void)seek_settle<FMT>(s, ix, q, false); }
+template <int FMT = 2>
+PA_HD void seek_complete2(Lane& s, const DevIndexView& ix, const SeekProbe& q0, bool two, const SeekProbe& q1) {
+    if (seek_settle<FMT>(s, ix, q0, two)) return;
+    (void)seek_settle<FMT>(s, ix, q1, false);
 }
 PA_HD void seek_finish(Lane& s, uint32_t K, uint32_t h, uint32_t off, bool full, uint32_t probe) {
     const uint32_t L = l_L(s), kp = l_kp(s);
@@ -595,6 +633,7 @@
                h1 = q.k1.x == q.w0 && q.k1.y == q.w1 && q.k1.z == q.w2 && q.k1.w == q.w3 && q.v1.x != NO_HANDLE;
     seek_finish(s, K, h0 ? q.v0.x : h1 ? q.v1.x : NO_HANDLE, h0 ? q.v0.y : q.v1.y, q.v0.x != NO_HANDLE && q.v1.x != NO_HANDLE, l_probe(s));
 }
+template <int FMT = 2>
 PA_HD void seek_step(Lane& s, const DevIndexView& ix, ReadRef rd) {
     const uint32_t K = ix.k;
     if (K > 32) {
@@ -605,9 +644,9 @@
     }
     SeekProbe q, q1;
     const bool two = seek_two(s, K);
-    seek_issue(s, ix, rd, q);
-    seek_issue(s, ix, rd, q1, PA_SEEK_STRIDE, two);
-    seek_complete2(s, K, q, two, q1);
+    seek_issue<FMT>(s, ix, rd, q);
+    seek_issue<FMT>(s, ix, rd, q1, PA_SEEK_STRIDE, two);
+    seek_complete2<FMT>(s, ix, q, two, q1);
 }
 #endif
 
diff --git a/rust-pseudoaligner_amd/csrc/map_pool.hip b/rust-pseudoaligner_amd/csrc/map_pool.hip
--- a/rust-pseudoaligner_amd/csrc/map_pool.hip
+++ b/rust-pseudoaligner_amd/csrc/map_pool.hip
@@ -50,6 +50,7 @@
     v.table = p->ix.table; v.nbuckets = p->ix.nbuckets; v.blobs = p->ix.blobs; v.ledge = p->ix.ledge;
     v.seg_g = p->ix.seg_g; v.seg_nid = p->ix.seg_nid; v.ec = p->ix.ec; v.class_ref = p->ix.class_ref; v.class_len = p->ix.class_len;
     v.wtable = p->ix.wtable; v.wbuckets = p->ix.wbuckets; v.kmask = p->ix.kmask; v.kmask_hi = p->ix.kmask_hi; v.k = p->ix.k; v.num_nodes = p->ix.num_nodes; v.num_classes = p->ix.num_classes; v.num_segs = p->ix.num_segs; v.stream_nt = p->ix.stream_nt; v.bitmap_min = p->ix.bitmap_min; v.bitmap_words = p->ix.bitmap_words;
+    v.dict_compact = p->ix.dict_compact; v.dict_w = p->ix.dict_w; v.dict_hbits = p->ix.dict_hbits;
     return v;
 }
 
@@ -264,12 +265,15 @@
     if (p.ix.k > 32)
         return p.pool_slots == 128 ? launch_kernel(&narrow::pa_map_pool_kernel<false, false, false, true, true>, p, grid, lds_bytes, stream)
                                    : launch_kernel(&narrow::pa_map_pool_kernel<false, false, false, false, true>, p, grid, lds_bytes, stream);
-    if (p.pool_slots == 128) return launch_kernel(&narrow::pa_map_pool_kernel<false, false, false, true>, p, grid, lds_bytes, stream);
-    return launch_kernel(&narrow::pa_map_pool_kernel<false, false, false, false>, p, grid, lds_bytes, stream);
+    if (p.ix.dict_compact)
+        return p.pool_slots == 128 ? launch_kernel(&narrow::pa_map_pool_kernel<false, false, false, true, false, 1>, p, grid, lds_bytes, stream)
+                                   : launch_kernel(&narrow::pa_map_pool_kernel<false, false, false, false, false, 1>, p, grid, lds_bytes, stream);
+    if (p.pool_slots == 128) return launch_kernel(&narrow::pa_map_pool_kernel<false, false, false, true, false, 0>, p, grid, lds_bytes, stream);
+    return launch_kernel(&narrow::pa_map_pool_kernel<false, false, false, false, false, 0>, p, grid, lds_bytes, stream);
 }
 
 int pool_kernel_occupancy(size_t lds_bytes, int* blocks_per_cu) {
-    return (int)hipOccupancyMaxActiveBlocksPerMultiprocessor(blocks_per_cu, reinterpret_cast<const void*>(&narrow::pa_map_pool_kernel<false, false, false, false>),
+    return (int)hipOccupancyMaxActiveBlocksPerMultiprocessor(blocks_per_cu, reinterpret_cast<const void*>(&narrow::pa_map_pool_kernel<false, false, false, false, false, 0>),
                                                              PA_MAP_BLOCK, lds_bytes);
 }
 
diff --git a/rust-pseudoaligner_amd/csrc/map_pool_kernel.inc b/rust-pseudoaligner_amd/csrc/map_pool_kernel.inc
--- a/rust-pseudoaligner_amd/csrc/map_pool_kernel.inc
+++ b/rust-pseudoaligner_amd/csrc/map_pool_kernel.inc
@@ -107,7 +107,7 @@
 #ifndef PA_MAP_MIN_BLOCKS
 #define PA_MAP_MIN_BLOCKS 3
 #endif
-template <bool TRACE, bool GREAD, bool DBG, bool S128 = false, bool KBIG = false>
+template <bool TRACE, bool GREAD, bool DBG, bool S128 = false, bool KBIG = false, int DFMT = 2>
 __global__ __launch_bounds__(PA_MAP_BLOCK, PA_MAP_MIN_BLOCKS) void pa_map_pool_kernel(const MapParams p_arg) {
     karg_ptr kp = (karg_ptr)__builtin_amdgcn_kernarg_segment_ptr();
     (void)p_arg;
@@ -269,7 +269,7 @@
             if (active) refill_slot<GREAD>(s, next + lane, slot, kp, rd, wc, S, wpr, K);
             next += n;
         } else if (sel == ST_SEEK) {
-            if (active) seek_step(s, ix, rr);
+            if (active) seek_step<DFMT>(s, ix, rr);
         } else if (sel == ST_FWD) {
             __builtin_amdgcn_s_waitcnt(0x0F70);
             Lane s2;
@@ -290,25 +290,25 @@
             SeekProbe pq;
             FwdLoad fl;
             PA_MARK("dual_state2");
-            pq.klo = pq.khi = pq.pending = 0; pq.v = U4{0u, 0u, NO_HANDLE, 0u};
+            seek_none<DFMT>(pq);
             SeekProbe2 pq2;
             if (KBIG) {
                 pq2.k0 = pq2.v0 = pq2.k1 = pq2.v1 = U4{0u, 0u, 0u, 0u}; pq2.v0.x = pq2.v1.x = NO_HANDLE; pq2.w0 = pq2.w1 = pq2.w2 = pq2.w3 = 0;
                 if (n2) seek_issue_k2(s2, ix, rr2, pq2);
             }
-            if (!KBIG && n2) seek_issue(s2, ix, rr2, pq);
+            if (!KBIG && n2) seek_issue<DFMT>(s2, ix, rr2, pq);
             const bool two_l = !KBIG && active2 && seek_two(s2, K);
             const bool pairs = __popcll(__ballot(two_l)) >= 8;
             const bool two = two_l && pairs;
             SeekProbe pq1;
-            pq1.klo = pq1.khi = pq1.pending = 0; pq1.v = U4{0u, 0u, NO_HANDLE, 0u};
-            if (pairs) seek_issue(s2, ix, rr2, pq1, PA_SEEK_STRIDE, two);
+            seek_none<DFMT>(pq1);
+            if (pairs) seek_issue<DFMT>(s2, ix, rr2, pq1, PA_SEEK_STRIDE, two);
             fwd_issue(s, ix, fl);
             __builtin_amdgcn_sched_barrier(0);
             PA_MARK("dual_issued");
             if (active2) {
                 if (KBIG) seek_complete_k2(s2, K, pq2);
-                else seek_complete2(s2, K, pq, two, pq1);
+                else seek_complete2<DFMT>(s2, ix, pq, two, pq1);
                 nq2 = queue_of(s2, K);
                 lane_store(s2, stA, stB, stC, slot2);
             }
```

Result: slower. 13.04 billion reads/s (-1.7%).
